# mueller-franzes/medfusion

Hardware: AMD Instinct MI355X
Metric: images/sec at 256x256, 150 DDIM steps (DiffusionPipeline.sample incl. VAE decode) (higher is better)
Workload: dtype f32 (emulated: fp16 pairs -- 23-bit operands, and 23-bit STORAGE of the tensors between the UNet's conv blocks: they exist as fp16 pairs only)

## Files before the change

### include/medfusion_hip.h

```cpp
#ifndef MEDFUSION_HIP_H
#define MEDFUSION_HIP_H

#include <stddef.h>
#include <stdint.h>

#ifdef __cplusplus
extern "C" {
#endif

#define MF_VERSION 250

enum { MF_OK = 0, MF_EINVAL = -1, MF_EUNSUPPORTED = -2, MF_ELAUNCH = -3, MF_EWORKSPACE = -4 };
enum { MF_LAYOUT_NHWC = 0, MF_LAYOUT_NCHW = 1 };

int mf_version(void);
const char* mf_last_error(void);

typedef struct MfConvDesc {
  int32_t N, Hin, Win;
  int32_t C1, C2;
  int32_t Cout;
  int32_t KH, KW;
  int32_t stride;
  int32_t pad;
  int32_t upsample;
  int32_t in_layout;
  int32_t out_layout;
  int32_t tile_hint;
  int32_t splitk_hint;
  int32_t precision;
} MfConvDesc;
enum { MF_CONV_FP32 = 0, MF_CONV_FP32_SPLIT3_W3 = 3, MF_CONV_BF16 = 4, MF_CONV_FP32_F16X2 = 5, MF_CONV_F16 = 6 };

int mf_pack_conv_weight_f32(const float* w_oihw, float* w_packed, int Cout, int Cin, int KH, int KW, void* stream);
int mf_pack_upconv_weight_f32(const float* w_oihw, float* w_packed, int Cout, int Cin, void* stream);
int mf_conv2d_subpixel_ok(const MfConvDesc* d);
int mf_conv2d_is_igemm(const MfConvDesc* d);
int mf_split_conv_weight_bf16x3(const float* w_packed, void* w_split, long rows, int K, void* stream);
int mf_convert_conv_weight_bf16(const float* w_packed, void* w_bf16, long rows, int K, void* stream);
size_t mf_conv2d_workspace_bytes(const MfConvDesc* d);
int mf_conv2d_f32(const float* x1, const float* x2, const float* w_packed, const float* bias, float* y,
                  void* workspace, size_t workspace_bytes, const MfConvDesc* d, void* stream);

int mf_conv2d_f16x2_ok(const MfConvDesc* d);
int mf_conv2d_f16x2_bound_slots(const MfConvDesc* d);
int mf_split_f16x2(const float* x, void* xs, const float* bound, int rows, int64_t per_row, void* stream);
int mf_split_f16x2_slots(const float* x, void* xs, const float* slots, int nslots, float* bound_out, int rows, int64_t per_row, void* stream);
int mf_conv2d_f16x2_sync_words(const MfConvDesc* d);
int mf_conv2d_f16x2(const void* x1s, const void* x2s, const void* ws, const float* bias, float* y, const float* x1_bound,
                    const float* x2_bound, float w_bound, float* y_bound, void* workspace, size_t workspace_bytes, uint32_t* sync,
                    double* gn_partial, int G, const MfConvDesc* d, void* stream);
int mf_conv2d_plan_query(const MfConvDesc* d, int32_t* tile_id, int32_t* splitk);
int mf_conv2d_plan_override(const MfConvDesc* d, int tile, int splitk);

typedef struct MfConvF16x2Call {
  const void* x1s; const void* x2s; const void* ws; const float* bias; float* y;
  const float* x1_bound; const float* x2_bound; float w_bound; float* y_bound;
  void* workspace; size_t workspace_bytes; uint32_t* sync;
  double* gn_partial; int G;
  const MfConvDesc* d;
} MfConvF16x2Call;
int mf_conv2d_f16x2_group_ok(const MfConvDesc* a, int Ga, const MfConvDesc* b, int Gb);
int mf_conv2d_f16x2_group(const MfConvF16x2Call* a, const MfConvF16x2Call* b, void* stream);

typedef struct MfGnFuse {
  const float* gamma;
  const float* beta;
  const float* residual;
  const void* residual_pairs;
  const float* res_bound;
  const float* res_bound_slots;
  const float* emb;
  const float* emb_bound;
  float* out;
  void* out_split;
  float* out_bound;
  uint32_t* rendezvous;
  uint32_t* error_flag;
  int64_t emb_stride;
  int32_t res_nslots;
  int32_t act;
  float bconst;
  float eps;
} MfGnFuse;
int mf_conv2d_f16x2_fuse_words(const MfConvDesc* d, int G);
int mf_conv2d_f16x2_gn_apply(const void* x1s, const void* x2s, const void* ws, const float* bias, const float* x1_bound, const float* x2_bound,
                             float w_bound, void* workspace, size_t workspace_bytes, uint32_t* sync, double* gn_partial, int G,
                             const MfGnFuse* f, const MfConvDesc* d, void* stream);

int mf_pack_nchw_pairs_f32(const float* x, void* out_pairs, float* bound_out, int N, int C, int HW, int CP, void* stream);
int mf_conv2d_f16x2_pairs_out_ok(const MfConvDesc* d);
int mf_conv2d_f16x2_pairs_out(const void* x1s, const void* x2s, const void* ws, const float* bias, float* y, void* y_split, float* y_bound_out,
                              const float* x1_bound, const float* x2_bound, float w_bound, float w_l1_1, float w_l1_2, float bias_max,
                              void* workspace, size_t workspace_bytes, uint32_t* sync, const MfConvDesc* d, void* stream);

int mf_wino_ok(const MfConvDesc* d);
int mf_wino_preferred(const MfConvDesc* d);
int mf_wino_in_table(const MfConvDesc* d);
int mf_wino_pack_weight_f32(const float* w_oihw, float* u, int Cout, int Cin, void* stream);
int mf_wino_input_f16x2(const void* xs, const float* x_bound, void* vs, float* v_bound, int N, int H, int W, int C, void* stream);
size_t mf_wino_workspace_bytes(const MfConvDesc* d);
int mf_wino_sync_words(const MfConvDesc* d);
int mf_wino_gn_parts(const MfConvDesc* d, int G);
int mf_wino_plan_query(const MfConvDesc* d, int32_t* tile_id, int32_t* splitk);
int mf_wino_f32_ok(const MfConvDesc* d, int G);
int mf_wino_input_f32(const float* x, float* v, int N, int H, int W, int C, void* stream);
int mf_wino_tail_f32(const float* m, const float* bias, const float* gamma, const float* beta, const float* residual, const float* emb, int64_t emb_stride,
                     float* out, float* out_wino, int N, int H, int W, int C, int G, int act, float eps, void* stream);
int mf_conv2d_wino_f16x2(const void* v1s, const void* v2s, const void* us, const float* bias, float* y, const float* v1_bound, const float* v2_bound,
                         float u_bound, void* workspace, size_t workspace_bytes, uint32_t* sync, double* gn_partial, int G, const MfConvDesc* d,
                         void* stream);
typedef struct MfWinoTail {
  const float* gamma; const float* beta;
  const float* residual; const void* residual_pairs;
  const float* res_bound; const float* res_bound_slots;
  const float* emb; const float* emb_bound;
  float* out; void* out_split; float* out_bound;
  void* out_wino; float* wino_bound;
  int64_t emb_stride;
  int32_t res_nslots, act;
  float bconst, eps;
} MfWinoTail;
int mf_wino_tail_ok(const MfConvDesc* d, int G);
int mf_wino_group_ok(const MfConvDesc* d, const MfConvDesc* guest);
int mf_conv2d_wino_gn_apply_f16x2(const void* v1s, const void* v2s, const void* us, const float* bias, const float* v1_bound, const float* v2_bound,
                                  float u_bound, void* workspace, size_t workspace_bytes, uint32_t* sync, int G, const MfWinoTail* t,
                                  const MfConvF16x2Call* guest, const MfConvDesc* d, void* stream);

int mf_conv2d_gn_parts(const MfConvDesc* d, int G);
int mf_conv2d_gn_f32(const float* x1, const float* x2, const float* w_packed, const float* bias, float* y, void* workspace,
                     size_t workspace_bytes, double* gn_partial, int G, const MfConvDesc* d, void* stream);

size_t mf_gn_stats_workspace_bytes(int N, int HW, int C, int G);
int mf_gn_stats_f32(const float* x, float* stats, void* workspace, size_t workspace_bytes, int N, int HW, int C, int G,
                    float eps, void* stream);
int mf_gn_partial_parts(int HW);
int mf_gn_stats_partial_f32(const float* x, double* partial, int N, int HW, int C, int G, void* stream);
int mf_gn_finalize_f32(const double* partial, int parts, float* stats, int N, int HW, int C, int G, float eps, void* stream);
int mf_gn_apply_f32(const float* x, const float* stats, const float* gamma, const float* beta, const float* residual,
                    const float* emb, int64_t emb_stride, float* out, int N, int HW, int C, int G, int act, void* stream);
int mf_gn_apply_split_f32(const float* x, const float* stats, const float* gamma, const float* beta, const float* residual,
                          const float* emb, int64_t emb_stride, float* out, void* out_split, const float* x_bound, const float* res_bound,
                          const float* emb_bound, float bconst, float* out_bound, int N, int HW, int C, int G, int act, void* stream);
int mf_gn_apply_from_partials_f32(const float* x, const double* gn_partial, int parts, float eps, const float* gamma, const float* beta,
                                  const float* residual, const float* emb, int64_t emb_stride, float* out, void* out_split,
                                  const float* res_bound, const float* res_bound_slots, int res_nslots, const float* emb_bound, float bconst,
                                  float* out_bound, int N, int HW, int C, int G, int act, void* stream);
int mf_gn_apply_from_partials_pairs_f32(const float* x, const double* gn_partial, int parts, float eps, const float* gamma, const float* beta,
                                        const float* residual, const void* residual_pairs, const float* emb, int64_t emb_stride, float* out,
                                        void* out_split, const float* res_bound, const float* res_bound_slots, int res_nslots,
                                        const float* emb_bound, float bconst, float* out_bound, int N, int HW, int C, int G, int act, void* stream);
int mf_maxabs_rows_slots(int64_t per_row);
int mf_maxabs_rows_f32(const float* x, float* partial, float* bound, int N, int64_t per_row, void* stream);
int mf_bound_finalize_f32(const float* partial, float* bound, int N, int slots, void* stream);

int mf_linear_f32(const float* x, int64_t x_stride, const float* w, const float* bias, float* y, int64_t y_stride,
                  int B, int In, int Out, int act_in, int act_out, int accumulate, void* stream);
int mf_sinusoidal_f32(const float* t, const float* freqs, float* out, int B, int dim, float max_period, float shift, int flip, void* stream);
int mf_learned_sinusoidal_f32(const float* t, const float* weights, float* out, int B, int emb_dim, void* stream);
int mf_embedding_add_f32(const float* table, const int64_t* idx, float* io, int B, int D, int num_rows, void* stream);

typedef struct MfSchedStep {
  float sqrt_recip_ac;
  float sqrt_recipm1_ac;
  float coef1, coef2;
  float std_fixed;
  float log_var_min;
  float log_var_max;
  float ddim_sqrt_an;
  float ddim_c;
  float ddim_sigma;
  int32_t t;
  int32_t mode;
} MfSchedStep;

typedef struct MfSchedArgs {
  const float* x_t;
  const float* pred;
  const float* pred_uncond;
  const float* pred_var;
  const float* noise_post;
  const float* noise_ddim;
  int64_t noise_step_stride;
  float* x_t_out;
  float* x0_out;
  float* xT_out;
  const MfSchedStep* table;
  const int32_t* step_dev;
  int32_t step;
  int32_t objective;
  int32_t clip_x0;
  float guidance_scale;
  int64_t n;
} MfSchedArgs;
int mf_sched_step_f32(const MfSchedArgs* a, void* stream);
int mf_sched_step_philox_f32(const MfSchedArgs* a, uint64_t seed, int32_t draw_base, int32_t draw_stride, int64_t sample_offset, int B,
                             int32_t* step_counter, uint32_t* ticket, void* stream);
typedef struct MfSchedBlend {
  const float* z0;
  const float* eps0;
  const uint8_t* mask;
  const float* coef;
  int64_t cells;
  int32_t channels;
  int32_t reserved;
} MfSchedBlend;
int mf_sched_step_blend_f32(const MfSchedArgs* a, const MfSchedBlend* blend, void* stream);
int mf_sched_step_philox_blend_f32(const MfSchedArgs* a, uint64_t seed, int32_t draw_base, int32_t draw_stride, int64_t sample_offset, int B,
                                   int32_t* step_counter, uint32_t* ticket, const MfSchedBlend* blend, void* stream);
enum { MF_SOLVER_FINAL = 0, MF_SOLVER_DDIM0 = 1, MF_SOLVER_ORDER1 = 2, MF_SOLVER_ORDER2 = 3 };
typedef struct MfSolverStep {
  float sqrt_recip_ac;
  float sqrt_recipm1_ac;
  float A, B, C;
  int32_t t;
  int32_t mode;
  int32_t reserved;
} MfSolverStep;
typedef struct MfSolverArgs {
  const float* x_t;
  const float* pred;
  const float* pred_uncond;
  float* x_t_out;
  float* x0_out;
  float* xT_out;
  float* x0_hist;
  const MfSolverStep* table;
  int32_t* step_counter;
  uint32_t* ticket;
  const int32_t* step_dev;
  int32_t step;
  int32_t objective;
  int32_t clip_x0;
  float guidance_scale;
  int64_t n;
} MfSolverArgs;
int mf_solver_step_f32(const MfSolverArgs* a, void* stream);
int mf_solver_step_blend_f32(const MfSolverArgs* a, const MfSchedBlend* blend, void* stream);
int mf_select_cells_f32(const uint8_t* mask, const float* a, const float* b, float* out, int N, int C, int64_t cells, void* stream);
int mf_mask_maxpool_u8(const void* mask, int mask_is_f32, uint8_t* out, int N, int D, int H, int W, int fd, int fh, int fw, void* stream);
int mf_broadcast_from_table_f32(const float* table, const int32_t* step_dev, int32_t step, float* out, int n, void* stream);
int mf_gather_step_rows_f32(const float* table, const int64_t* cols, const int32_t* step_dev, int32_t step, int ncol, int64_t row_len,
                            float* out, int B, void* stream);
int mf_gather_step_rows3_f32(const float* const* tables, const int64_t* row_lens, float* const* outs, int n_tables, const int64_t* cols,
                             const int32_t* step_dev, int32_t step, int ncol, int B, void* stream);
int mf_counter_add_i32(int32_t* counter, int32_t inc, void* stream);

int mf_rows_axpby_f32(const float* x, const float* y, const float* a, const float* c, const float* d, float* out, int B,
                      int64_t per_row, int do_clamp, float lo, float hi, void* stream);

int mf_philox_normal_f32(float* out, uint64_t seed, int32_t draw_base, int32_t draw_stride, const int32_t* step_dev,
                         int32_t step, int64_t sample_offset, int B, int64_t per_sample, void* stream);

int mf_attention_f32(const float* q, const float* k, const float* v, float* out, int B, int H, int Nq, int Nk, int d,
                     float scale, void* stream);
int mf_layernorm_f32(const float* x, const float* gamma, const float* beta, float* out, int64_t rows, int C, float eps,
                     void* stream);
int mf_geglu_f32(const float* h, float* out, int64_t rows, int C, void* stream);
int mf_add_f32(const float* a, const float* b, float* out, int64_t n, void* stream);

int mf_nchw_to_nhwc_f32(const float* x, float* y, int N, int C, int H, int W, void* stream);
int mf_nhwc_to_nchw_f32(const float* x, float* y, int N, int C, int H, int W, void* stream);
int mf_diag_gaussian_sample_f32(const float* moments, const float* noise, float* z, int N, int C, int HW, void* stream);
int mf_diag_gaussian_kl_f32(const float* moments, float* kl, int N, int C, int HW, void* stream);

size_t mf_vq_workspace_bytes(int64_t pixels);
int mf_vector_quantize_f32(const float* z, const float* codebook, float* z_q, int32_t* idx, double* sqerr, void* workspace,
                           size_t workspace_bytes, int N, int C, int HW, int K, void* stream);

typedef struct MfConv3dDesc {
  int32_t N, D, H, W;
  int32_t C1, C2;
  int32_t Cout;
  int32_t k;
  int32_t stride[3];
  int32_t pad[3];
  int32_t upsample[3];
  int32_t tile_hint;
  int32_t splitk_hint;
  int32_t precision;
// ... 40 lines not shown
```

### medfusion_amd/blocks.py

```python
from __future__ import annotations

import os
from typing import Optional, Tuple, Union

import torch
import torch.nn as nn

from . import kernels as K
from . import lib as L

Act = Union[torch.Tensor, Tuple[torch.Tensor, torch.Tensor]]


def monai_padding(kernel_size: int, stride: int) -> int:
    p = (kernel_size - stride + 1) / 2
    if p < 0:
        raise AssertionError("padding value should not be negative")
    return int(p)


def zero_module(m: nn.Module) -> nn.Module:
    for p in m.parameters():
        p.detach().zero_()
    return m


def _split(x: Act):
    return (x[0], x[1]) if isinstance(x, (tuple, list)) else (x, None)


class _Packed:

    def __init__(self, subpixel: bool = False, pad_cin: int = 0):
        self._pad_cin = pad_cin
        self._key = None
        self._w = None
        self._w3 = None
        self._wb = None
        self._wh = None
        self._wu = None
        self._l1 = {}
        self._subpixel = subpixel

    def get(self, weight: torch.Tensor) -> torch.Tensor:
        key = (weight.data_ptr(), weight._version, weight.device)
        if key != self._key:
            w = weight.detach()
            if w.dim() == 3:
                w = w.unsqueeze(-1)
            if self._pad_cin and w.shape[1] < self._pad_cin:
                w = torch.nn.functional.pad(w, (0, 0, 0, 0, 0, self._pad_cin - w.shape[1]))
            self._w = K.pack_upconv_weight(w) if self._subpixel else K.pack_conv_weight(w)
            self._w3 = None
            self._wb = None
            self._wh = None
            self._wu = None
            self._l1 = {}
            self._raw = w
            self._key = key
        return self._w

    def get_wino(self, weight: torch.Tensor):
        self.get(weight)
        if self._wu is None:
            self._wu = K.split_weight_f16x2(K.wino_pack_weight(self._raw))
        return self._wu

    def get_wino_f32(self, weight: torch.Tensor, split3: bool):
        self.get(weight)
        if getattr(self, "_wuf_key", None) != self._key:
            self._wuf, self._wu3, self._wuf_key = K.wino_pack_weight(self._raw), None, self._key
        if not split3:
            return self._wuf
        if self._wu3 is None:
            self._wu3 = K.split_conv_weight(self._wuf)
        return self._wu3

    def get_f16x2(self, weight: torch.Tensor) -> torch.Tensor:
        wp = self.get(weight)
        if self._wh is None:
            self._wh = K.split_weight_f16x2(wp)
        return self._wh

    def l1(self, weight: torch.Tensor, c1: int):
        wp = self.get(weight)
        ent = self._l1.get(c1)
        if ent is None:
            a = wp[..., :c1].abs().sum(dim=(-3, -2, -1)).max()
            b = wp[..., c1:].abs().sum(dim=(-3, -2, -1)).max() if c1 < wp.shape[-1] else torch.zeros((), device=wp.device)
            ent = self._l1[c1] = (float(a.item()) * (1.0 + 1e-5), float(b.item()) * (1.0 + 1e-5))
        return ent

    def get_bf16(self, weight: torch.Tensor) -> torch.Tensor:
        wp = self.get(weight)
        if self._wb is None:
            self._wb = K.convert_conv_weight_bf16(wp)
        return self._wb

    def get_split(self, weight: torch.Tensor) -> torch.Tensor:
        wp = self.get(weight)
        if self._w3 is None:
            self._w3 = K.split_conv_weight(wp)
        return self._w3


PAIRS_ONLY_BETWEEN_BLOCKS = os.environ.get("MEDFUSION_PAIRS_ONLY", "1") != "0"
INPUT_CONV_ON_PAIRS = os.environ.get("MEDFUSION_INPUT_CONV_PAIRS", "0") == "1"
GROUPED_CONV_RES = os.environ.get("MEDFUSION_GROUPED_CONV_RES", "1") != "0"
GROUP_GUEST = {}
DERIVED_OUT_BOUNDS = os.environ.get("MEDFUSION_DERIVED_BOUNDS", "1") != "0"
SUBPIXEL_UPSAMPLE = True
CONV_PRECISION = int(os.environ.get("MEDFUSION_CONV_PRECISION", "5"))
WINOGRAD = int(os.environ.get("MEDFUSION_WINOGRAD", "1"))


WINOGRAD_F32 = int(os.environ.get("MEDFUSION_WINOGRAD_F32", "1"))
WINOGRAD_F32_MFMA = int(os.environ.get("MEDFUSION_WINOGRAD_F32_MFMA", "0"))
WINO_TAIL = os.environ.get("MEDFUSION_WINOGRAD_TAIL", "1") != "0"
WINO_GROUP = os.environ.get("MEDFUSION_WINOGRAD_GROUP", "1") != "0"
WINO_SHAPES = {}
if os.environ.get("MEDFUSION_WINOGRAD_TABLE"):
    import json as _json
    WINO_SHAPES = {tuple(e[:5]): (int(e[5]), int(e[6])) for e in _json.load(open(os.environ["MEDFUSION_WINOGRAD_TABLE"]))}


def wino_wanted(d) -> bool:
    if WINOGRAD == 0:
        return False
    if (d.N, d.Hin, d.Win, d.C1 + d.C2, d.Cout) in WINO_SHAPES:
        return K.wino_ok(d)
    return K.wino_ok(d) if WINOGRAD == 2 else K.wino_preferred(d)


def f16x2_mode() -> bool:
    return CONV_PRECISION in (5, 6)


class Conv(nn.Module):

    def __init__(self, in_ch, out_ch, kernel_size, stride=1, padding=0, upsample=False, conv1d=False):
        super().__init__()
        holder = nn.Conv1d(in_ch, out_ch, 1) if conv1d else nn.Conv2d(in_ch, out_ch, kernel_size, stride, padding, bias=True)
        self.weight, self.bias = holder.weight, holder.bias
        self.in_ch, self.out_ch, self.k, self.stride, self.pad, self.upsample = in_ch, out_ch, kernel_size, stride, padding, int(upsample)
        self._packed = _Packed()
        self._packed_sub = _Packed(subpixel=True)
        self._packed_pad = _Packed(pad_cin=32)
        self._pad_ok = {}
        self._descs = {}
        self._pairs_out = {}
        self._wino_sites = {}
        self._bmax = (None, 0.0)

    def _forward_f16x2(self, x1, x2, n, h, w, c1, c2, out, gn_groups, gn_eps, measure_out, prec=5, derive_out=False, cin_pad=0):
        key = ("f16x2", n, h, w, c1, c2, gn_groups, prec, WINOGRAD)
        ent = self._descs.get(key)
        if ent is None:
            d = K.make_conv_desc(n, h, w, c1, c2, self.out_ch, self.k, self.stride, self.pad, 2 if self.upsample else 0, precision=prec)
            ok = K.conv_f16x2_ok(d)
            pinned = K.pin_conv_plan(d) if ok else None
            wino = None
            if ok and prec == 5 and not cin_pad and self.k == 3 and wino_wanted(d):
                wparts = K.wino_gn_parts(d, gn_groups) if gn_groups else 0
                if not gn_groups or wparts > 0:
                    wt, wsk = WINO_SHAPES.get((n, h, w, c1 + c2, self.out_ch), (0, 0))
                    wd = K.make_conv_desc(n, h, w, c1, c2, self.out_ch, self.k, self.stride, self.pad, 0, tile_hint=wt, splitk_hint=wsk, precision=prec)
                    wino = (wd, wparts, K.pin_wino_plan(wd))
            ent = (d, K.conv_gn_parts(d, gn_groups) if (ok and gn_groups) else 0, ok, pinned, wino)
            self._descs[key] = ent
        d, parts, ok, pinned, wino = ent
        if not ok:
            return None
        if wino is not None and out is None and not measure_out and not derive_out:
            wd, wparts, wpinned = wino
            r = K.conv2d_wino_f16x2(x1, self._packed.get_wino(self.weight), self.bias, wd, x2=x2, gn_groups=gn_groups, gn_parts=wparts, pinned=wpinned)
            return (r[0], K.GnPartials(r[1], wparts, gn_eps)) if gn_groups else r
        pk = self._packed_pad if cin_pad else (self._packed_sub if d.upsample == 2 else self._packed)
        wh = pk.get_f16x2(self.weight)
        if not gn_groups:
            if derive_out and out is None and DERIVED_OUT_BOUNDS:
                po = self._pairs_out.get(key)
                if po is None:
                    po = self._pairs_out[key] = K.conv_pairs_out_ok(d)
                if po:
                    bkey = (self.bias._version, self.bias.data_ptr())
                    if self._bmax[0] != bkey:
                        self._bmax = (bkey, float(self.bias.detach().abs().max().item()))
                    return K.conv2d_f16x2_pairs_out(x1, wh, self.bias, d, pk.l1(self.weight, c1), self._bmax[1], x2=x2, pinned=pinned)
            return K.conv2d_f16x2(x1, wh, self.bias, d, x2=x2, out=out, measure_out=measure_out, pinned=pinned)
        ho, wo = K.conv_out_hw(d)
        if parts > 0:
            y, partial = K.conv2d_f16x2(x1, wh, self.bias, d, x2=x2, out=out, gn_groups=gn_groups, gn_parts=parts, pinned=pinned)
        else:
            y = K.conv2d_f16x2(x1, wh, self.bias, d, x2=x2, out=out, pinned=pinned)
            partial, parts = K.gn_stats_partial(y, gn_groups)
        if gn_groups <= 256:
            return y, K.GnPartials(partial, parts, gn_eps)
        return y, K.gn_finalize(partial, parts, ho * wo, self.out_ch, gn_groups, gn_eps)

    def wino_tail_desc(self, x: Act, G: int):
        x1, x2 = _split(x)
        n, h, w, c1 = x1.shape
        c2 = 0 if x2 is None else x2.shape[-1]
        key = ("wino_tail", n, h, w, c1, c2, G, WINOGRAD, WINO_TAIL)
        ent = self._descs.get(key)
        if ent is None:
            ent = False
            if WINO_TAIL and CONV_PRECISION == 5 and self.k == 3 and self.stride == 1 and not self.upsample and c1 + c2 == self.in_ch:
                d = K.make_conv_desc(n, h, w, c1, c2, self.out_ch, self.k, self.stride, self.pad, 0, precision=5)
                if wino_wanted(d) and K.wino_tail_ok(d, G):
                    wt, wsk = WINO_SHAPES.get((n, h, w, c1 + c2, self.out_ch), (0, 0))
                    d.tile_hint, d.splitk_hint = wt, wsk
                    ent = (d, K.pin_wino_plan(d))
            self._descs[key] = ent
        return (key, ent) if ent is not False else (key, None)

    def forward_wino_gn_apply(self, x: Act, norm, act: int, residual, emb, emb_stride, out_fp32, bconst, guest=None):
        x1, x2 = _split(x)
        n, h, w, c1 = x1.shape
        c2 = 0 if x2 is None else x2.shape[-1]
        if c1 + c2 != self.in_ch:
            raise RuntimeError(f"conv expects {self.in_ch} input channels, got {c1}+{c2}")
        G = norm.num_groups
        key, ent = self.wino_tail_desc(x, G)
        if ent is None:
            return None
        d, pinned = ent
        want = self._wino_sites.get(key, False)
        y = K.conv2d_wino_gn_apply(x1, self._packed.get_wino(self.weight), self.bias, d, norm.weight, norm.bias, G, norm.eps, act=act, residual=residual,
                                   emb=emb, emb_stride=emb_stride, x2=x2, bconst=bconst, out_fp32=out_fp32, want_wino=want, pinned=pinned, guest=guest)
        if not want:
            y._mf_wino_site = (self._wino_sites, key)
        return y

    def forward_wino_gn_apply_f32(self, x: Act, norm, act: int, residual, emb, emb_stride, split3: bool = True):
        x1, x2 = _split(x)
        n, h, w, c1 = x1.shape
        c2 = 0 if x2 is None else x2.shape[-1]
        G = norm.num_groups
        mode = WINOGRAD_F32 if split3 else WINOGRAD_F32_MFMA
        key = ("wino_f32", n, h, w, c1, c2, G, mode, split3)
        ent = self._descs.get(key)
        if ent is None:
            ent = False
            if self.k == 3 and self.stride == 1 and not self.upsample and c1 + c2 == self.in_ch:
                d = K.make_conv_desc(n, h, w, c1, c2, self.out_ch, 3, 1, 1, 0, precision=3 if split3 else 0)
                if K.wino_f32_ok(d, G) and K.conv_is_igemm(d):
                    rule = K.make_conv_desc(n, h, w, c1, c2, self.out_ch, 3, 1, 1, 0, precision=5)
                    if mode == 2 or h * w <= 256 or K.wino_preferred(rule):
                        ent = d
            self._descs[key] = ent
        if ent is False:
            return None
        K._need_f32(x1, x2, residual)
        want = self._wino_sites.get(key, False)
        y = K.conv2d_wino_gn_apply_f32(x1, self._packed.get_wino_f32(self.weight, split3), self.bias, ent, norm.weight, norm.bias, G, norm.eps, act=act,
                                       residual=residual, emb=emb, emb_stride=emb_stride, x2=x2, want_wino=want)
        if not want:
            y._mf_wino_site_f32 = (self._wino_sites, key)
        return y

    def forward_gn_apply(self, x: Act, norm, act: int, residual, emb, emb_stride, out_fp32, bconst):
        x1, x2 = _split(x)
        n, h, w, c1 = x1.shape
        c2 = 0 if x2 is None else x2.shape[-1]
        if c1 + c2 != self.in_ch:
            raise RuntimeError(f"conv expects {self.in_ch} input channels, got {c1}+{c2}")
        prec = CONV_PRECISION
        G = norm.num_groups
        key = ("fused", n, h, w, c1, c2, G, prec)
        ent = self._descs.get(key)
        if ent is None:
# ... 547 lines not shown
```

### medfusion_amd/csrc/conv_f16x2.h

```cpp
#pragma once
#include "common.h"
#include "split_f16.h"

#ifndef MFC2_HZ
#define MFC2_HZ 0
#endif
#ifndef MFC2_OUT_STORE
#define MFC2_OUT_STORE 0
#endif

namespace mfc2 {
using namespace mf;

typedef float f32x16 __attribute__((ext_vector_type(16)));
typedef float f32x4 __attribute__((ext_vector_type(4)));
typedef unsigned int u32x4 __attribute__((ext_vector_type(4)));
typedef _Float16 f16x8 __attribute__((ext_vector_type(8)));
typedef _Float16 f16x2 __attribute__((ext_vector_type(2)));

struct FuseP {
  int on, act;
  float eps, bconst;
  double count;
  const float* gamma;
  const float* beta;
  const float* res_f32;
  const void* res_pairs;
  const float* res_bound;
  const float* res_slots;
  int res_nslots;
  int tiles_per_sample;
  const float* emb;
  long emb_stride;
  const float* emb_bound;
  float* out_f32;
  void* out_pairs;
  float* out_bound;
  unsigned* rv;
  unsigned* rv_err;
};

struct ConvP2 {
  const void* x1;
  const void* x2;
  const void* w;
  const float* bias;
  float* y;
  const float* bound1;
  const float* bound2;
  int wexp;
  float* out_bound;
  int bound_slots;
  int N, Hin, Win, C1, C2, Cin, Cout;
  int Hout, Wout, Heff, Weff, KH, KW, stride, pad;
  int M, K, HWout;
  int cgroups, cg_per_split, splitk;
  int tiles_m, tiles_n;
  long slab;
  unsigned bytes1, bytes2, bytesw;
  int subpix, hw_src;
  int out_nt;
  int wphase_rows;
  int walk_n_fast;
  double* gn_partial;
  int gn_groups, gn_parts, gn_cpg;
  int tree;
  float* handoff;
  unsigned* sync;
  FuseP fz;
  void* y_pairs;
  float* y_pair_bound;
  float wl1_1, wl1_2, bmax;
#if MFC2_HZ & (256 | 512)
  float* dbg;
#endif
};

__device__ __forceinline__ int xcd_remap2(int bid, int total) {
  const int q = total >> 3, r = total & 7;
  const int xcd = bid & 7, within = bid >> 3;
  const int base = xcd < r ? xcd * (q + 1) : r * (q + 1) + (xcd - r) * q;
  return base + within;
}

#ifndef MFC2_HZ
#define MFC2_HZ 0
#endif
#define MFC2_HZ_ON(BIT) ((MFC2_HZ >> (BIT)) & 1)
#ifndef MFC2_HZ_PAD
#define MFC2_HZ_PAD 7
#endif

__device__ __forceinline__ float hz_add(float a, float b) { float r; asm volatile("v_add_f32 %0, %1, %2" : "=v"(r) : "v"(a), "v"(b)); return r; }
__device__ __forceinline__ float hz_mul(float a, float b) { float r; asm volatile("v_mul_f32 %0, %1, %2" : "=v"(r) : "v"(a), "v"(b)); return r; }

#define MFC2_WAIT_VM(N) asm volatile("s_waitcnt vmcnt(%0)" ::"n"(N) : "memory")
#if MFC2_HZ & 512
#define MFC2_STAMP(I) { if (p.dbg && threadIdx.x == 0) reinterpret_cast<unsigned long*>(p.dbg)[(long)MFC2_BID * 8 + (I)] = __builtin_amdgcn_s_memrealtime(); }
#else
#define MFC2_STAMP(I)
#endif
#define MFC2_WAIT_LGKM0() asm volatile("s_waitcnt lgkmcnt(0)" ::: "memory")

#define MFC2_BODY_AS_KERNEL 1
#define MFC2_BID blockIdx.x
#include "conv_f16x2_body.inc"
#undef MFC2_BODY_AS_KERNEL
#undef MFC2_BID
#define MFC2_BODY_AS_KERNEL 0
#define MFC2_BID bid
#include "conv_f16x2_body.inc"
#undef MFC2_BODY_AS_KERNEL
#undef MFC2_BID

__global__ __launch_bounds__(256) void split_act_f16x2_kernel(const float* __restrict__ x, u32x4* __restrict__ out, long octets,
                                                              const float* __restrict__ bound, long octets_per_row) {
  const long stride = (long)gridDim.x * blockDim.x;
  for (long o = (long)blockIdx.x * blockDim.x + threadIdx.x; o < octets; o += stride) {
    const float sc = bound ? exp2i(-scale_exp_of(bound[o / octets_per_row])) : 1.f;
    const f32x4 v0 = *reinterpret_cast<const f32x4*>(x + o * 8) * sc, v1 = *reinterpret_cast<const f32x4*>(x + o * 8 + 4) * sc;
    u32x4 hi, lo;
    split8_f16(v0, v1, hi, lo);
    out[o * 2] = hi;
    out[o * 2 + 1] = lo;
  }
}

__global__ __launch_bounds__(256) void split_act_slots_kernel(const float* __restrict__ x, u32x4* __restrict__ out, long octets_per_row,
                                                              const float* __restrict__ slots, int nslots, float* __restrict__ bound_out) {
  __shared__ float sm[4];
  const int row = blockIdx.y, tid = threadIdx.x;
  float m = 0.f;
  for (int i = tid; i < nslots; i += 256) m = fmaxf(m, slots[(long)row * nslots + i]);
  m = mf::wave_max(m);
  if ((tid & 63) == 0) sm[tid >> 6] = m;
  __syncthreads();
  const float b = fmaxf(fmaxf(sm[0], sm[1]), fmaxf(sm[2], sm[3]));
  if (blockIdx.x == 0 && tid == 0) bound_out[row] = b;
  const float sc = exp2i(-scale_exp_of(b));
  const long base = (long)row * octets_per_row;
  for (long o = (long)blockIdx.x * 256 + tid; o < octets_per_row; o += (long)gridDim.x * 256) {
    const f32x4 v0 = *reinterpret_cast<const f32x4*>(x + (base + o) * 8) * sc, v1 = *reinterpret_cast<const f32x4*>(x + (base + o) * 8 + 4) * sc;
    u32x4 hi, lo;
    split8_f16(v0, v1, hi, lo);
    out[(base + o) * 2] = hi;
    out[(base + o) * 2 + 1] = lo;
  }
}

}
```

### medfusion_amd/csrc/conv_f16x2.hip

```cpp
#include "common.h"
#include <string.h>
#include <mutex>
#include <vector>
#include "gn_partial.h"
#include "conv_plan.h"
#include "conv_f16x2.h"
#include "conv_f16x2_halo.h"
#include "conv_f16x2_group.h"
#include "winograd.h"

using namespace mf;

namespace {

struct Tile2 { int id, BM, BN, WM, WN, NST, HG; };
const Tile2 kTiles2[] = {
    {31, 128, 256, 2, 4, 3, 0}, {32, 256, 128, 4, 2, 3, 0}, {33, 128, 128, 2, 4, 3, 0}, {34, 128, 128, 4, 2, 3, 0}, {35, 256, 64, 4, 2, 3, 0},
    {36, 128, 64, 4, 2, 3, 0}, {37, 64, 256, 1, 8, 3, 0},
    {51, 128, 128, 2, 2, 2, 0}, {52, 128, 128, 2, 2, 3, 0}, {53, 64, 128, 2, 2, 3, 0}, {54, 128, 64, 2, 2, 3, 0},
    {61, 256, 128, 4, 2, 3, 6}, {62, 256, 128, 4, 2, 3, 7}, {63, 128, 128, 2, 4, 3, 4}, {64, 128, 128, 2, 4, 3, 5},
};
inline size_t tile_lds(const Tile2& t) {
  return t.HG ? (size_t)2 * t.HG * (t.WM * t.WN) * 1024 + (size_t)3 * t.BN * 128 : (size_t)t.NST * (t.BM + t.BN) * 128;
}
// ... 305 lines not shown
}

static int bound_slots2(const MfConvDesc* d, const Plan2& pl, bool with_stats) {
  const int HW = pl.Hout * pl.Wout;
  if (pl.splitk == 1 || tree_possible(d, pl)) {
    if (!tile_sample_aligned(pl)) return 0;
    const int nw = pl.t.WM * pl.t.WN;
    return HW >= pl.t.BM ? (HW / pl.t.BM) * (d->Cout / pl.t.BN) * nw : (d->Cout / pl.t.BN) * (nw * HW / pl.t.BM);
  }
  if (with_stats) return 0;
  const long p4 = (long)HW * d->Cout / 4;
  int bx = (int)((p4 + 255) / 256);
  const int cap = cdiv(2048, d->N);
  if (bx > cap) bx = cap;
  return bx * 4;
}

int mf_conv2d_f16x2_bound_slots(const MfConvDesc* d) {
  Plan2 pl;
  if (!d || !pair_precision(d->precision) || make_plan2(d, &pl) != MF_OK || !pl.ok) return 0;
  return bound_slots2(d, pl, false);
}

int mf_conv2d_plan_query(const MfConvDesc* d, int32_t* tile_id, int32_t* splitk) {
  MF_REQUIRE(d, MF_EINVAL, "plan_query: null desc");
  if (pair_precision(d->precision)) {
    Plan2 pl;
    int rc = make_plan2(d, &pl);
    if (rc) return rc;
    if (tile_id) *tile_id = pl.ok ? pl.t.id : 0;
    if (splitk) *splitk = pl.ok ? pl.splitk : 0;
    return MF_OK;
  }
  return igemm_plan_query(d, tile_id, splitk);
}

int mf_split_f16x2(const float* x, void* xs, const float* bound, int rows, int64_t per_row, void* stream) {
  MF_REQUIRE(x && xs && rows > 0 && per_row > 0 && per_row % 8 == 0, MF_EINVAL, "split_f16x2: bad args (per_row %% 8 == 0)");
  const long octets = (long)rows * (per_row / 8);
  ProfScope ps(MF_FAM_MISC, (hipStream_t)stream, 0, 8.0 * rows * (double)per_row);
  const int blocks = (int)((octets + 255) / 256 > 8192 ? 8192 : (octets + 255) / 256);
  MF_LAUNCH(mfc2::split_act_f16x2_kernel, dim3(blocks), dim3(256), 0, (hipStream_t)stream, x, reinterpret_cast<mfc2::u32x4*>(xs), octets, bound,
                     (long)(per_row / 8));
  return check_launch("split_f16x2");
}

int mf_split_f16x2_slots(const float* x, void* xs, const float* slots, int nslots, float* bound_out, int rows, int64_t per_row, void* stream) {
  MF_REQUIRE(x && xs && slots && bound_out && nslots > 0 && rows > 0 && rows <= 65535 && per_row > 0 && per_row % 8 == 0, MF_EINVAL,
             "split_f16x2_slots: bad args (per_row %% 8 == 0, rows <= 65535)");
  const long opr = per_row / 8;
  ProfScope ps(MF_FAM_MISC, (hipStream_t)stream, 0, 8.0 * rows * (double)per_row);
  long bpr = (opr + 255) / 256;
  const long cap = (8192 + rows - 1) / rows;
  if (bpr > cap) bpr = cap;
  MF_LAUNCH(mfc2::split_act_slots_kernel, dim3((int)bpr, rows), dim3(256), 0, (hipStream_t)stream, x, reinterpret_cast<mfc2::u32x4*>(xs), opr, slots, nslots,
            bound_out);
  return check_launch("split_f16x2_slots");
}

static int host_scale_exp(float bound) {
  if (!(bound > 0.f)) return 0;
  uint32_t u;
  memcpy(&u, &bound, 4);
  const int s = (int)((u >> 23) & 0xffu) - 127 - 14;
  return s < -100 ? -100 : (s > 100 ? 100 : s);
}

int mf_conv2d_plan_override(const MfConvDesc* d, int tile, int splitk) {
  MF_REQUIRE(d && pair_precision(d->precision), MF_EINVAL, "plan_override: a MF_CONV_FP32_F16X2 / MF_CONV_F16 descriptor");
  std::lock_guard<std::mutex> lk(g_plan_mu);
  const int Cin = d->C1 + d->C2;
  for (size_t i = 0; i < g_plan_overrides.size(); ++i) {
    const PlanEntry& e = g_plan_overrides[i];
    if (e.N == d->N && e.H == d->Hin && e.W == d->Win && e.Cin == Cin && e.Cout == d->Cout && e.k == d->KH && e.stride == d->stride && e.ups == d->upsample) {
      g_plan_overrides.erase(g_plan_overrides.begin() + i);
      break;
    }
  }
  if (tile > 0 && splitk > 0) g_plan_overrides.push_back(PlanEntry{d->N, d->Hin, d->Win, Cin, d->Cout, d->KH, d->stride, d->upsample, tile, splitk});
  return MF_OK;
}

int mf_conv2d_f16x2_sync_words(const MfConvDesc* d) {
  Plan2 pl;
  if (!d || !pair_precision(d->precision) || make_plan2(d, &pl) != MF_OK || !pl.ok || !tree_possible(d, pl)) return 0;
  return cdiv(pl.M, pl.t.BM) * (d->Cout / pl.t.BN) * (pl.splitk - 1);
}

static int fuse_tiles_per_sample(const MfConvDesc* d, const Plan2& pl, int G) {
  if (!pl.ok || G <= 0 || G > 256 || d->Cout % G || d->upsample != 0) return 0;
  if (pl.splitk > 1 && !tree_possible(d, pl)) return 0;
  if (!epilogue_stats_ok(d, pl, G)) return 0;
  const int HW = pl.Hout * pl.Wout;
  if (HW < pl.t.BM && pl.t.BM / HW > 8) return 0;
  const long grid = (long)cdiv(pl.M, pl.t.BM) * (d->Cout / pl.t.BN) * pl.splitk;
  mfc2::ConvP2 dummy{};
  const int resident = dispatch_tile(pl.t.id, dummy, nullptr, d->precision == MF_CONV_F16 ? 1 : 3, 1);
  if (resident <= 0 || grid > resident) return 0;
  static const int fault = [] { const char* e = getenv("MEDFUSION_FUSE_FAULT"); return e ? atoi(e) : 0; }();
  return (HW >= pl.t.BM ? HW / pl.t.BM : 1) * (d->Cout / pl.t.BN) + (fault ? 1 : 0);
}

int mf_conv2d_f16x2_fuse_words(const MfConvDesc* d, int G) {
  Plan2 pl;
  if (!d || !pair_precision(d->precision) || make_plan2(d, &pl) != MF_OK || !pl.ok) return 0;
  return fuse_tiles_per_sample(d, pl, G) > 0 ? 2 * d->N : 0;
}

struct PairsOut { void* y_split; float* y_bound; float wl1_1, wl1_2, bmax; };
static int conv_f16x2_impl(const void* x1s, const void* x2s, const void* ws, const float* bias, float* y, const float* x1_bound, const float* x2_bound,
                           float w_bound, float* y_bound, void* workspace, size_t workspace_bytes, uint32_t* sync, double* gn_partial, int G,
                           const MfGnFuse* fz, const MfConvDesc* d, void* stream, const PairsOut* po = nullptr);

int mf_conv2d_f16x2_pairs_out_ok(const MfConvDesc* d) {
  Plan2 pl;
  if (!d || !pair_precision(d->precision) || make_plan2(d, &pl) != MF_OK || !pl.ok || d->Cout % 8) return 0;
  return (pl.splitk == 1 || tree_possible(d, pl)) ? 1 : 0;
}

int mf_conv2d_f16x2_pairs_out(const void* x1s, const void* x2s, const void* ws, const float* bias, float* y, void* y_split, float* y_bound_out,
                              const float* x1_bound, const float* x2_bound, float w_bound, float w_l1_1, float w_l1_2, float bias_max, void* workspace,
                              size_t workspace_bytes, uint32_t* sync, const MfConvDesc* d, void* stream) {
  MF_REQUIRE(y && y_split && y_bound_out && x1_bound, MF_EINVAL, "conv(f16x2, pairs out): y, y_split, y_bound_out and x1_bound are required");
  MF_REQUIRE(d && (d->C2 == 0 || x2_bound), MF_EINVAL, "conv(f16x2, pairs out): x2_bound with a second source");
  MF_REQUIRE(mf_conv2d_f16x2_pairs_out_ok(d), MF_EUNSUPPORTED, "conv(f16x2, pairs out): this plan reduces split-K behind the launch (mf_conv2d_f16x2_pairs_out_ok == 0)");
  MF_REQUIRE(w_l1_1 >= 0.f && w_l1_2 >= 0.f && bias_max >= 0.f, MF_EINVAL, "conv(f16x2, pairs out): norms must be >= 0");
  const PairsOut po{y_split, y_bound_out, w_l1_1, w_l1_2, bias_max};
  return conv_f16x2_impl(x1s, x2s, ws, bias, y, x1_bound, x2_bound, w_bound, nullptr, workspace, workspace_bytes, sync, nullptr, 0, nullptr, d, stream, &po);
}

int mf_conv2d_f16x2(const void* x1s, const void* x2s, const void* ws, const float* bias, float* y, const float* x1_bound, const float* x2_bound,
                    float w_bound, float* y_bound, void* workspace, size_t workspace_bytes, uint32_t* sync, double* gn_partial, int G,
                    const MfConvDesc* d, void* stream) {
  MF_REQUIRE(y, MF_EINVAL, "conv(f16x2): null pointer");
  return conv_f16x2_impl(x1s, x2s, ws, bias, y, x1_bound, x2_bound, w_bound, y_bound, workspace, workspace_bytes, sync, gn_partial, G, nullptr, d, stream);
}

int mf_conv2d_f16x2_gn_apply(const void* x1s, const void* x2s, const void* ws, const float* bias, const float* x1_bound, const float* x2_bound,
                             float w_bound, void* workspace, size_t workspace_bytes, uint32_t* sync, double* gn_partial, int G, const MfGnFuse* f,
                             const MfConvDesc* d, void* stream) {
  MF_REQUIRE(f && gn_partial && G > 0, MF_EINVAL, "conv_gn_apply: needs the fuse arguments, the record array and G");
  MF_REQUIRE(f->out_split && f->out_bound && f->rendezvous && f->error_flag, MF_EINVAL, "conv_gn_apply: out_split, out_bound, rendezvous and error_flag are required");
  MF_REQUIRE((f->gamma == nullptr) == (f->beta == nullptr), MF_EINVAL, "conv_gn_apply: gamma/beta must both be given or both NULL");
  MF_REQUIRE(!(f->residual && f->residual_pairs), MF_EINVAL, "conv_gn_apply: the residual is fp32 OR fp16 pairs");
  MF_REQUIRE(!f->residual_pairs || f->res_bound, MF_EINVAL, "conv_gn_apply: a residual given as fp16 pairs needs the res_bound that scaled it");
  MF_REQUIRE(!f->residual || f->res_bound || (f->res_bound_slots && f->res_nslots > 0), MF_EINVAL, "conv_gn_apply: a residual needs res_bound or res_bound_slots");
  MF_REQUIRE(!f->emb || (f->emb_bound && f->emb_stride % 4 == 0), MF_EINVAL, "conv_gn_apply: an embedding needs emb_bound and emb_stride %% 4 == 0");
  return conv_f16x2_impl(x1s, x2s, ws, bias, nullptr, x1_bound, x2_bound, w_bound, nullptr, workspace, workspace_bytes, sync, gn_partial, G, f, d, stream);
}

struct Prep { mfc2::ConvP2 p; Plan2 pl; bool tree; double flops, bytes; int terms; };
static int conv_f16x2_prepare(const void* x1s, const void* x2s, const void* ws, const float* bias, float* y, const float* x1_bound, const float* x2_bound,
                              float w_bound, float* y_bound, void* workspace, size_t workspace_bytes, uint32_t* sync, double* gn_partial, int G,
                              const MfGnFuse* fz, const MfConvDesc* d, const PairsOut* po, Prep* out, bool wino_gemm = false) {
  MF_REQUIRE(d && pair_precision(d->precision), MF_EINVAL, "conv(f16x2): desc.precision must be MF_CONV_FP32_F16X2 (or the opt-in MF_CONV_F16)");
  MF_REQUIRE((d->upsample == 3) == wino_gemm, MF_EINVAL, "conv(f16x2): upsample = 3 is internal to mf_conv2d_wino_f16x2");
  Plan2& pl = out->pl;
  mfc2::ConvP2& p = out->p;
  int rc = make_plan2(d, &pl);
  if (rc) return rc;
  MF_REQUIRE(pl.ok, MF_EUNSUPPORTED, "conv(f16x2): this shape/layout is not on the fp16-pair path (ask mf_conv2d_f16x2_ok)");
  MF_REQUIRE(x1s && ws && (y || fz), MF_EINVAL, "conv(f16x2): null pointer");
  MF_REQUIRE(d->C2 == 0 || x2s != nullptr, MF_EINVAL, "conv(f16x2): C2 > 0 but x2 is null");
  MF_REQUIRE(!gn_partial || gn_parts2(d, pl, G) > 0, MF_EUNSUPPORTED, "conv(f16x2): cannot emit GroupNorm partials (mf_conv2d_gn_parts == 0)");
  MF_REQUIRE(!y_bound || (!gn_partial && bound_slots2(d, pl, false) > 0), MF_EUNSUPPORTED,
             "conv(f16x2): cannot measure the output bound of this plan (mf_conv2d_f16x2_bound_slots == 0, or GroupNorm statistics requested)");
  p.x1 = x1s; p.x2 = x2s; p.w = ws; p.bias = bias; p.y = y;
  p.bound1 = x1_bound; p.bound2 = x2_bound; p.wexp = host_scale_exp(w_bound); p.out_bound = y_bound; p.bound_slots = y_bound ? bound_slots2(d, pl, false) : 0;
  p.N = d->N; p.Hin = d->Hin; p.Win = d->Win; p.C1 = d->C1; p.C2 = d->C2; p.Cin = d->C1 + d->C2; p.Cout = d->Cout;
  p.Hout = pl.Hout; p.Wout = pl.Wout; p.Heff = pl.Heff; p.Weff = pl.Weff;
  p.KH = d->KH; p.KW = d->KW; p.stride = d->stride; p.pad = d->pad;
  p.subpix = d->upsample == 2 ? 1 : 0; p.hw_src = d->Hin * d->Win;
  if (p.subpix) { p.KH = p.KW = 2; p.Heff = d->Hin; p.Weff = d->Win; }
  p.M = pl.M; p.K = pl.K; p.HWout = pl.Hout * pl.Wout;
  p.cgroups = pl.cgroups; p.cg_per_split = pl.cg_per_split; p.splitk = pl.splitk;
  p.tiles_m = cdiv(pl.M, pl.t.BM); p.tiles_n = d->Cout / pl.t.BN;
  p.slab = (long)pl.M * d->Cout;
  p.bytes1 = (unsigned)(4.0 * d->N * d->Hin * d->Win * d->C1);
  p.bytes2 = (unsigned)(4.0 * d->N * d->Hin * d->Win * d->C2);
  p.bytesw = (unsigned)(4.0 * d->Cout * pl.K * (p.subpix ? 4 : wino_gemm ? 16 : 1));
  p.wphase_rows = wino_gemm ? (d->N / 16) * d->Hin * d->Win : 0;
  {
    static const int walk = [] { const char* e = getenv("MF_CONV_WALK"); return e ? atoi(e) : 1; }();
    const double act_bytes = 4.0 * d->N * d->Hin * d->Win * (d->C1 + d->C2), w_bytes = 4.0 * d->Cout * pl.K * (p.subpix ? 4 : 1);
    p.walk_n_fast = (!wino_gemm && p.tiles_n > 1 && (walk == 2 || (walk == 1 && act_bytes > w_bytes))) ? 1 : 0;
  }
  p.out_nt = 0;
  p.gn_partial = nullptr; p.gn_groups = G; p.gn_cpg = G > 0 ? d->Cout / G : 8; p.gn_parts = 0;
  p.tree = 0; p.handoff = nullptr; p.sync = nullptr;
#if MFC2_HZ & (256 | 512)
  p.dbg = g_conv_dbg;
#endif
  p.y_pairs = po ? po->y_split : nullptr; p.y_pair_bound = po ? po->y_bound : nullptr;
  p.wl1_1 = po ? po->wl1_1 : 0.f; p.wl1_2 = po ? po->wl1_2 : 0.f; p.bmax = po ? po->bmax : 0.f;
  memset(&p.fz, 0, sizeof(p.fz));
  if (fz) {
    const int tps = fuse_tiles_per_sample(d, pl, G);
    MF_REQUIRE(tps > 0, MF_EUNSUPPORTED, "conv_gn_apply: this plan cannot apply its GroupNorm inside the launch (mf_conv2d_f16x2_fuse_words == 0)");
    p.fz.on = 1; p.fz.act = fz->act; p.fz.eps = fz->eps; p.fz.bconst = fz->bconst; p.fz.count = (double)(pl.Hout * pl.Wout) * (d->Cout / G);
    p.fz.gamma = fz->gamma; p.fz.beta = fz->beta; p.fz.res_f32 = fz->residual; p.fz.res_pairs = fz->residual_pairs;
    p.fz.res_bound = fz->res_bound; p.fz.res_slots = fz->res_bound ? nullptr : fz->res_bound_slots; p.fz.res_nslots = fz->res_nslots;
    p.fz.tiles_per_sample = tps; p.fz.emb = fz->emb; p.fz.emb_stride = (long)fz->emb_stride; p.fz.emb_bound = fz->emb_bound;
    p.fz.out_f32 = fz->out; p.fz.out_pairs = fz->out_split; p.fz.out_bound = fz->out_bound; p.fz.rv = fz->rendezvous; p.fz.rv_err = fz->error_flag;
  }
  const bool tree = pl.splitk > 1 && tree_possible(d, pl) && (!gn_partial || epilogue_stats_ok(d, pl, G));
  if ((pl.splitk == 1 || tree) && gn_partial) { p.gn_partial = gn_partial; p.gn_parts = p.HWout >= pl.t.BM ? p.HWout / pl.t.BM : 1; }
  if (tree) {
    const size_t need = tree_handoff_bytes(d, pl);
    MF_REQUIRE(workspace && workspace_bytes >= need, MF_EWORKSPACE, "conv(f16x2): workspace %zu < %zu", workspace_bytes, need);
    MF_REQUIRE(sync, MF_EINVAL, "conv(f16x2): this plan meets its split-K slices inside the launch and needs `sync` "
                                "(mf_conv2d_f16x2_sync_words(d) zero-initialised words the caller keeps between launches)");
    p.tree = tree_mode(); p.handoff = reinterpret_cast<float*>(workspace); p.sync = sync;
    if (y_bound && p.bound_slots == 0) p.out_bound = nullptr;
  } else if (pl.splitk > 1) {
    const size_t need = (size_t)pl.splitk * pl.M * d->Cout * sizeof(float);
    MF_REQUIRE(workspace && workspace_bytes >= need, MF_EWORKSPACE, "conv(f16x2): workspace %zu < %zu", workspace_bytes, need);
    p.y = reinterpret_cast<float*>(workspace);
    p.out_bound = nullptr;
  }
  out->tree = tree;
  out->flops = 2.0 * pl.M * (double)d->Cout * (d->upsample == 2 ? 9.0 * (d->C1 + d->C2) : (double)pl.K);
  out->bytes = 4.0 * ((double)d->N * d->Hin * d->Win * p.Cin + (double)d->Cout * pl.K + (double)pl.M * d->Cout);
  out->terms = d->precision == MF_CONV_F16 ? 1 : 3;
  return MF_OK;
}

static int conv_f16x2_impl(const void* x1s, const void* x2s, const void* ws, const float* bias, float* y, const float* x1_bound, const float* x2_bound,
                           float w_bound, float* y_bound, void* workspace, size_t workspace_bytes, uint32_t* sync, double* gn_partial, int G,
                           const MfGnFuse* fz, const MfConvDesc* d, void* stream, const PairsOut* po) {
  Prep q;
  int rc = conv_f16x2_prepare(x1s, x2s, ws, bias, y, x1_bound, x2_bound, w_bound, y_bound, workspace, workspace_bytes, sync, gn_partial, G, fz, d, po, &q);
  if (rc) return rc;
  hipStream_t s = (hipStream_t)stream;
  const Plan2& pl = q.pl;
  const mfc2::ConvP2& p = q.p;
  const bool tree = q.tree;
  {
    const int terms = q.terms;
    ProfScope ps(fz ? MF_FAM_CONV_GN_FUSED : MF_FAM_CONV_IGEMM, s, q.flops, q.bytes, 2.0 * pl.M * (double)d->Cout * pl.K * terms);
    ps.set_tag(pl.t.id + (terms == 1 ? 100000 : 0));
    rc = dispatch_tile(pl.t.id, p, s, terms, 0);
    if (rc == -1) { set_error("conv(f16x2): no tile config %d", pl.t.id); rc = MF_EINVAL; }
  }
  if (rc) return rc;
  if (pl.splitk > 1 && !tree) {
    const int HW = p.HWout;
    ProfScope ps(MF_FAM_SPLITK_REDUCE, s, 0, 4.0 * pl.M * d->Cout * (pl.splitk + 1));
    if (gn_partial) {
      const int slices = stats_slices(d->N, HW, d->Cout, G), chunks = stats_chunks(HW);
      MF_LAUNCH(gn_partial_kernel<true>, dim3(chunks, d->N, slices), dim3(kStatsThreads), stats_lds_bytes(d->Cout / slices), s,
                         reinterpret_cast<const float*>(workspace), gn_partial, HW, d->Cout, G, pl.splitk, p.slab, bias, y, (float*)nullptr);
      return check_launch("splitk_reduce_stats");
    }
    const long p4 = (long)HW * d->Cout / 4;
    int bx = (int)((p4 + 255) / 256);
    const int cap = cdiv(2048, d->N);
    if (bx > cap) bx = cap;
    MF_LAUNCH(splitk_reduce_kernel<0>, dim3(bx, d->N), dim3(256), 0, s, reinterpret_cast<const float*>(workspace), bias, y, p4, d->Cout,
                       pl.splitk, p.slab, y_bound);
    return check_launch("splitk_reduce");
  }
  return MF_OK;
}

static bool single_launch(const MfConvDesc* d, const Plan2& pl, int G) {
  if (pl.splitk == 1) return G == 0 || gn_parts2(d, pl, G) > 0;
  return tree_possible(d, pl) && (G == 0 || epilogue_stats_ok(d, pl, G));
}

int mf_conv2d_f16x2_group_ok(const MfConvDesc* a, int Ga, const MfConvDesc* b, int Gb) {
  static const int off = [] { const char* e = getenv("MF_CONV_GROUP"); return e && atoi(e) == 0 ? 1 : 0; }();
  if (off || !a || !b || a->precision != MF_CONV_FP32_F16X2 || b->precision != MF_CONV_FP32_F16X2) return 0;
  Plan2 pa, pb;
  if (make_plan2(a, &pa) != MF_OK || make_plan2(b, &pb) != MF_OK || !pa.ok || !pb.ok) return 0;
  if (!single_launch(a, pa, Ga) || !single_launch(b, pb, Gb)) return 0;
  mfc2::ConvP2 dummy{};
  return dispatch_group(pa.t.id, pb.t.id, dummy, dummy, nullptr, 2) == 1 ? 1 : 0;
}

int mf_conv2d_f16x2_group(const MfConvF16x2Call* a, const MfConvF16x2Call* b, void* stream) {
  MF_REQUIRE(a && b && a->d && b->d && a->y && b->y, MF_EINVAL, "conv_group: two calls with descriptors and outputs");
  const int Ga = a->gn_partial ? a->G : 0, Gb = b->gn_partial ? b->G : 0;
  MF_REQUIRE(mf_conv2d_f16x2_group_ok(a->d, Ga, b->d, Gb), MF_EUNSUPPORTED,
             "conv_group: these two plans cannot share a launch (mf_conv2d_f16x2_group_ok == 0: a reducer pass behind one of them, workgroup sizes "
             "that differ, or a tile pair that is not instantiated)");
  Prep qa, qb;
  int rc = conv_f16x2_prepare(a->x1s, a->x2s, a->ws, a->bias, a->y, a->x1_bound, a->x2_bound, a->w_bound, a->y_bound, a->workspace, a->workspace_bytes,
                              a->sync, a->gn_partial, a->G, nullptr, a->d, nullptr, &qa);
  if (rc) return rc;
  rc = conv_f16x2_prepare(b->x1s, b->x2s, b->ws, b->bias, b->y, b->x1_bound, b->x2_bound, b->w_bound, b->y_bound, b->workspace, b->workspace_bytes,
                          b->sync, b->gn_partial, b->G, nullptr, b->d, nullptr, &qb);
  if (rc) return rc;
  MF_REQUIRE((qa.pl.splitk == 1 || qa.tree) && (qb.pl.splitk == 1 || qb.tree), MF_EUNSUPPORTED, "conv_group: a plan needs its reducer pass");
  if (qa.tree && qb.tree) {
    const char *wa = (const char*)a->workspace, *wb = (const char*)b->workspace;
    const size_t na = tree_handoff_bytes(a->d, qa.pl), nb = tree_handoff_bytes(b->d, qb.pl);
    MF_REQUIRE(wa + na <= wb || wb + nb <= wa, MF_EINVAL, "conv_group: the two workspaces overlap");
    const uint32_t *sa = a->sync, *sb = b->sync;
    const long ca = mf_conv2d_f16x2_sync_words(a->d), cb = mf_conv2d_f16x2_sync_words(b->d);
    MF_REQUIRE(sa + ca <= sb || sb + cb <= sa, MF_EINVAL, "conv_group: the two sync arrays overlap");
  }
  MF_REQUIRE(a->y != b->y, MF_EINVAL, "conv_group: one output for two convolutions");
  hipStream_t s = (hipStream_t)stream;
  ProfScope ps(MF_FAM_CONV_IGEMM, s, qa.flops + qb.flops, qa.bytes + qb.bytes,
               2.0 * 3.0 * (qa.pl.M * (double)a->d->Cout * qa.pl.K + qb.pl.M * (double)b->d->Cout * qb.pl.K));
  ps.set_tag(1000 + 100 * qa.pl.t.id + qb.pl.t.id);
  rc = dispatch_group(qa.pl.t.id, qb.pl.t.id, qa.p, qb.p, s, 0);
  if (rc == -1) { set_error("conv_group: no tile pair (%d, %d)", qa.pl.t.id, qb.pl.t.id); rc = MF_EINVAL; }
  return rc;
}

int mf_prof_tag_name(int family, int tag, char* buf, int n) {
  MF_REQUIRE(buf && n > 0, MF_EINVAL, "mf_prof_tag_name: bad args");
  auto tile_of = [](int id) -> const Tile2* { for (const auto& k : kTiles2) if (k.id == id) return &k; return nullptr; };
  auto tile_type = [&](int id, char* o, int m) {
    const Tile2* t = tile_of(id);
    if (!t) { snprintf(o, m, "?"); return; }
    if (t->HG) snprintf(o, m, "mfc2::HaloTile<%d, %d, %d, %d, %d>", t->BM, t->BN, t->WM, t->WN, t->HG);
    else snprintf(o, m, "mfc2::PlainTile<%d, %d, %d, %d, %d>", t->BM, t->BN, t->WM, t->WN, t->NST);
  };
  if ((family == MF_FAM_CONV_IGEMM || family == MF_FAM_CONV_GN_FUSED) && tag > 0) {
    const int terms = tag >= 100000 ? 1 : 3, id = tag % 100000;
    if (id >= 1000) {
      char a[96], b[96];
      tile_type((id - 1000) / 100, a, sizeof a);
      tile_type((id - 1000) % 100, b, sizeof b);
      snprintf(buf, n, "void mfc2::conv_group_kernel<%s, %s, 3>(mfc2::ConvP2, mfc2::ConvP2, int)", a, b);
      return MF_OK;
    }
    if (const Tile2* t = tile_of(id)) {
      if (t->HG) snprintf(buf, n, "void mfc2::conv_halo_kernel<%d, %d, %d, %d, %d, %d>(mfc2::ConvP2)", t->BM, t->BN, t->WM, t->WN, t->HG, terms);
      else snprintf(buf, n, "void mfc2::conv_f16x2_kernel<%d, %d, %d, %d, %d, %d>(mfc2::ConvP2)", t->BM, t->BN, t->WM, t->WN, t->NST, terms);
      return MF_OK;
    }
// ... 9 lines not shown
```

### medfusion_amd/csrc/conv_f16x2_body.inc

```
template <int BM, int BN, int WM, int WN, int NST, int TERMS = 3>
#if MFC2_BODY_AS_KERNEL
__global__ __launch_bounds__(WM * WN * 64, 2) void conv_f16x2_kernel(const ConvP2 p) {
#else
__device__ __forceinline__ void conv_f16x2_body(const ConvP2& p, const int bid) {
#endif
  static_assert(TERMS == 3 || TERMS == 1, "three product terms (fp16 pairs) or one (fp16)");
  constexpr int PC = TERMS == 3 ? 2 : 1;
  constexpr int NW = WM * WN;
  static_assert(NW == 8 || NW == 4, "4 or 8 waves");
  constexpr int FM = BM / WM, FN = BN / WN, TM = FM / 32, TN = FN / 32;
  static_assert(TM >= 1 && TN >= 1 && FM % 32 == 0 && FN % 32 == 0, "per-wave footprint");
  constexpr int GP = BM / (8 * NW), GQ = BN / (8 * NW), NL = GP + GQ;
  static_assert(BM % (8 * NW) == 0 && BN % (8 * NW) == 0, "tile");
  constexpr int ROWB = 128, STAGE = (BM + BN) * ROWB;
  constexpr int NM = TERMS * TM * TN;
  constexpr int NR = PC * (TM + TN);
  constexpr int NF = (2 * NM + 2) / 3;
  static_assert(NST >= 2 && NST <= 6 && NST * STAGE <= 160 * 1024 && (NST - 1) * NL <= 63, "LDS stages");
  static_assert((NR + NF - 1) / NF <= 3, "at most three reads per slot");

  extern __shared__ __attribute__((aligned(1024))) char smem[];
  MFC2_STAMP(0)

  const int tid = threadIdx.x, lane = tid & 63;
  const int wave = __builtin_amdgcn_readfirstlane(tid >> 6);
  const int wm = wave / WN, wn = wave % WN;

  const int total = p.tiles_m * p.tiles_n * p.splitk;
  const int logical = xcd_remap2(MFC2_BID, total);
  int tile_m = logical % p.tiles_m;
  const int rest = logical / p.tiles_m;
  int tile_n = rest % p.tiles_n;
  int kz = rest / p.tiles_n;
  if (p.walk_n_fast) {
    tile_n = logical % p.tiles_n;
    const int r1 = logical / p.tiles_n;
    tile_m = r1 % p.tiles_m;
    kz = r1 / p.tiles_m;
  }
  if (p.wphase_rows) {
    const int tpc = p.wphase_rows / BM, ncomp = p.tiles_m / tpc;
    const int tm_in = logical % tpc, r1 = logical / tpc;
    tile_n = r1 % p.tiles_n;
    const int r2 = r1 / p.tiles_n;
    tile_m = (r2 % ncomp) * tpc + tm_in;
    kz = r2 / ncomp;
  }
  const int m0 = tile_m * BM, n0 = tile_n * BN;
  const int cg_beg = kz * p.cg_per_split;
  const int cg_end = min(p.cgroups, cg_beg + p.cg_per_split);
  const int taps = p.KH * p.KW;
  const int nit = (cg_end - cg_beg) * taps;

  const int lrow = lane >> 3;
  const unsigned slot16 = (unsigned)(((lane & 7) ^ ((4 * (wave & 1) + (lane >> 4)) & 7)) * 16);
  int a_pix[GP], a_inv[GP];
  const bool small_m = p.M < (1 << 23);
  const float r_hw = 1.0f / (float)p.HWout, r_w = 1.0f / (float)(p.subpix ? p.Win : p.Wout), r_src = 1.0f / (float)p.hw_src;
  auto qdiv = [small_m](int a, int d, float rd) {
    if (!small_m) return a / d;
    int q = (int)((float)a * rd);
    const int r = a - q * d;
    q += (r >= d ? 1 : 0) - (r < 0 ? 1 : 0);
    return q;
  };
#pragma unroll
  for (int i = 0; i < GP; ++i) {
    const int m = m0 + 8 * (wave + NW * i) + lrow;
    int n_ = 0, iy0 = -(1 << 28), ix0 = 0;
    if (m < p.M) {
      const int n = qdiv(m, p.HWout, r_hw);
      const int rem = m - n * p.HWout;
      n_ = n * p.Hin;
      if (p.subpix) {
        const int ph = qdiv(rem, p.hw_src, r_src), r2 = rem - ph * p.hw_src;
        const int y = qdiv(r2, p.Win, r_w), x = r2 - y * p.Win;
        iy0 = y + (ph >> 1) - 1;
        ix0 = x + (ph & 1) - 1;
      } else {
        const int oy = qdiv(rem, p.Wout, r_w), ox = rem - oy * p.Wout;
        iy0 = oy * p.stride - p.pad;
        ix0 = ox * p.stride - p.pad;
      }
    }
    unsigned vy = 0, vx = 0;
#pragma unroll
    for (int t = 0; t < 3; ++t) {
      vy |= (t < p.KH && (unsigned)(iy0 + t) < (unsigned)p.Heff ? 1u : 0u) << t;
      vx |= (t < p.KW && (unsigned)(ix0 + t) < (unsigned)p.Weff ? 1u : 0u) << t;
    }
    const unsigned valid = ((vy & 1u) ? vx : 0u) | ((vy & 2u) ? vx << p.KW : 0u) | ((vy & 4u) ? vx << (2 * p.KW) : 0u);
    a_inv[i] = (int)~valid;
    a_pix[i] = (n_ + iy0) * p.Win + ix0;
  }
  const __amdgpu_buffer_rsrc_t rsw = __builtin_amdgcn_make_buffer_rsrc(const_cast<void*>(p.w), 0, p.bytesw, 0x00020000);
  const int phase_t = p.subpix ? ((m0 % p.HWout) / p.hw_src) : (p.wphase_rows ? m0 / p.wphase_rows : 0);
  const unsigned kbytes = (unsigned)p.K * 4u;
  const unsigned qv = (unsigned)(phase_t * p.Cout + n0 + 8 * wave + lrow) * kbytes + slot16;

  int l_cc = cg_beg, l_ky = 0, l_kx = 0, l_it = 0, l_st = 0;
  unsigned pbase[GP], l_off[GP];
  unsigned l_cs4 = 0, l_so = 0;
  int l_lds = 0;
  __amdgpu_buffer_rsrc_t l_rs = rsw;

#define MFC2_CHUNK_SETUP()                                                                                              \
  {                                                                                                                     \
    const int c0_ = l_cc * 32;                                                                                          \
    const bool first_ = c0_ < p.C1;                                                                                     \
    l_cs4 = (unsigned)(first_ ? p.C1 : p.C2) * 4u;                                                                      \
    const unsigned cb4_ = (unsigned)(first_ ? c0_ : c0_ - p.C1) * 4u + slot16;                                          \
    l_rs = __builtin_amdgcn_make_buffer_rsrc(const_cast<void*>(first_ ? p.x1 : p.x2), 0, first_ ? p.bytes1 : p.bytes2, 0x00020000); \
    _Pragma("unroll") for (int i = 0; i < GP; ++i) pbase[i] = (unsigned)a_pix[i] * l_cs4 + cb4_;                        \
  }
#define MFC2_LOAD_PREP()                                                                                                \
  {                                                                                                                     \
    const unsigned ts_ = (unsigned)(l_ky * p.KW + l_kx);                                                                \
    const unsigned tapb_ = (unsigned)(l_ky * p.Win + l_kx) * l_cs4;                                                     \
    _Pragma("unroll") for (int i = 0; i < GP; ++i) l_off[i] = (pbase[i] + tapb_) | (unsigned)__builtin_amdgcn_sbfe(a_inv[i], ts_, 1u); \
    l_so = (ts_ * (unsigned)p.Cin + (unsigned)l_cc * 32u) * 4u;                                                         \
    l_lds = l_st * STAGE + wave * 1024;                                                                                 \
  }
#define MFC2_LOAD_UNIT(U)                                                                                               \
  {                                                                                                                     \
    constexpr int u_ = (U);                                                                                             \
    if constexpr (u_ < GP) {                                                                                            \
      const unsigned off_ = l_off[u_];    \
      __builtin_amdgcn_raw_ptr_buffer_load_lds(l_rs, (__attribute__((address_space(3))) void*)(smem + l_lds + NW * u_ * 1024), 16, off_, 0, 0, 0); \
    } else {                                                                                                            \
      constexpr int q_ = u_ - GP;                                                                                       \
      __builtin_amdgcn_raw_ptr_buffer_load_lds(rsw, (__attribute__((address_space(3))) void*)(smem + l_lds + BM * ROWB + NW * q_ * 1024), 16, qv, \
                                               l_so + (unsigned)q_ * (8u * NW) * kbytes, 0, 0);                         \
    }                                                                                                                   \
  }
#define MFC2_LOAD_ADVANCE()                  \
  {                                          \
    ++l_it;                                  \
    l_st = l_st == NST - 1 ? 0 : l_st + 1;   \
    ++l_kx;                                  \
    if (l_kx == p.KW) { l_kx = 0; ++l_ky; }  \
    if (l_ky == p.KH) {                      \
      l_ky = 0;                              \
      ++l_cc;                                \
      if (l_it < nit) MFC2_CHUNK_SETUP()     \
    }                                        \
  }
#define MFC2_LOAD_ALL()                                            \
  {                                                                \
    MFC2_LOAD_PREP()                                               \
    MFC2_LOAD_UNIT(0) MFC2_LOAD_UNIT(1)                            \
    if constexpr (NL > 2) MFC2_LOAD_UNIT(NL > 2 ? 2 : 0)           \
    if constexpr (NL > 3) MFC2_LOAD_UNIT(NL > 3 ? 3 : 0)           \
    if constexpr (NL > 4) MFC2_LOAD_UNIT(NL > 4 ? 4 : 0)           \
    if constexpr (NL > 5) MFC2_LOAD_UNIT(NL > 5 ? 5 : 0)           \
    if constexpr (NL > 6) MFC2_LOAD_UNIT(NL > 6 ? 6 : 0)           \
    if constexpr (NL > 7) MFC2_LOAD_UNIT(NL > 7 ? 7 : 0)           \
  }

  const int fkey = (lane >> 1) & 7, fh = lane >> 5;
  int foff[2][2];
#pragma unroll
  for (int s = 0; s < 2; ++s)
#pragma unroll
    for (int c = 0; c < 2; ++c) foff[s][c] = (lane & 31) * ROWB + (((4 * s + 2 * fh + c) ^ fkey) * 16);
  const int xrow0 = wm * FM * ROWB;
  const int wrow0 = BM * ROWB + wn * FN * ROWB;

  f32x16 accm[TM][TN], accx[TM][TN];
#pragma unroll
  for (int i = 0; i < TM; ++i)
#pragma unroll
    for (int j = 0; j < TN; ++j)
#pragma unroll
      for (int r = 0; r < 16; ++r) { accm[i][j][r] = 0.f; accx[i][j][r] = 0.f; }

  f16x8 fx[2][TM][2], fw[2][TN][2];

  const bool first_src1 = cg_beg * 32 < p.C1, last_src2 = (cg_end - 1) * 32 >= p.C1;
  const int it_sw = __builtin_amdgcn_readfirstlane((first_src1 && last_src2) ? (p.C1 / 32 - cg_beg) * taps : -1);
#ifndef MFC2_EXPS_EARLY
#define MFC2_EXPS_EARLY 1
#endif
#if MFC2_EXPS_EARLY
#define MFC2_PIXEL_EXPS_DECL()                                                                                          \
  float pb1[TM] = {}, pb2[TM] = {};    \
  f32x4 eb0 = {0.f, 0.f, 0.f, 0.f}, eb1 = {0.f, 0.f, 0.f, 0.f};
#define MFC2_PIXEL_EXPS_LOAD()                                                                                          \
  _Pragma("unroll") for (int i = 0; i < TM; ++i) {                                                                      \
    const int pm_ = min(m0 + wm * FM + i * 32 + (lane & 31), p.M - 1);                                                  \
    const int pn_ = pm_ / p.HWout;                                                                                      \
    pb1[i] = p.bound1 ? p.bound1[pn_] : 0.f;                                                                            \
    pb2[i] = (p.bound2 && p.C2 > 0) ? p.bound2[pn_] : 0.f;                                                              \
  }                                                                                                                     \
  if ((p.splitk == 1 || p.tree) && p.bias) {                                                                            \
    const int bc0_ = n0 + wn * FN + (lane % (FN / 8)) * 8;                                                              \
    eb0 = *reinterpret_cast<const f32x4*>(p.bias + bc0_);                                                               \
    eb1 = *reinterpret_cast<const f32x4*>(p.bias + bc0_ + 4);                                                           \
  }
#define MFC2_PIXEL_EXPS(I) const int e1_ = p.bound1 ? scale_exp_of(pb1[I]) : 0, e2_ = (p.bound2 && p.C2 > 0) ? scale_exp_of(pb2[I]) : 0;
#else
#define MFC2_PIXEL_EXPS_DECL()
#define MFC2_PIXEL_EXPS_LOAD()
#define MFC2_PIXEL_EXPS(I)                                                                                              \
    const int pm_ = min(m0 + wm * FM + (I) * 32 + (lane & 31), p.M - 1);                                                \
    const int pn_ = pm_ / p.HWout;                                                                                      \
    const int e1_ = p.bound1 ? scale_exp_of(p.bound1[pn_]) : 0;                                                         \
    const int e2_ = (p.bound2 && p.C2 > 0) ? scale_exp_of(p.bound2[pn_]) : 0;
#endif
  MFC2_PIXEL_EXPS_DECL()
#define MFC2_SOURCE_SWITCH()                                                                                            \
  if (__builtin_expect(it == it_sw, 0)) {                                                                               \
    if constexpr (MFC2_HZ_ON(0)) asm volatile("s_nop 15\n\ts_nop 15" ::: "memory");                                     \
    _Pragma("unroll") for (int i = 0; i < TM; ++i) {                                                                    \
      MFC2_PIXEL_EXPS(i)                                                                                                \
      const float f_ = exp2i(e1_) * exp2i(-e2_);                                                                        \
      _Pragma("unroll") for (int j = 0; j < TN; ++j)                                                                    \
        _Pragma("unroll") for (int r = 0; r < 16; ++r) { accm[i][j][r] *= f_; accx[i][j][r] *= f_; }                    \
    }                                                                                                                   \
  }

#define MFC2_READ_UNIT(S, SB, U)                                                                                        \
  {                                                                                                                     \
    constexpr int u_ = (U);                                                                                             \
    if constexpr (u_ < PC * TM) {                                                                                       \
      fx[S][u_ / PC][u_ % PC] = *reinterpret_cast<const f16x8*>(smem + (SB) + xrow0 + (u_ / PC) * 32 * ROWB + foff[S][u_ % PC]); \
    } else {                                                                                                            \
      constexpr int v_ = u_ - PC * TM;                                                                                  \
      fw[S][v_ / PC][v_ % PC] = *reinterpret_cast<const f16x8*>(smem + (SB) + wrow0 + (v_ / PC) * 32 * ROWB + foff[S][v_ % PC]); \
    }                                                                                                                   \
  }
#define MFC2_MFMA(S, N_)                                                                                                \
  {                                                                                                                     \
    constexpr int n_ = (N_);                                                                                            \
    constexpr int j_ = n_ % TN, i_ = (n_ / TN) % TM, t_ = n_ / (TN * TM);                                               \
    if constexpr (t_ == 0) accm[i_][j_] = __builtin_amdgcn_mfma_f32_32x32x16_f16(fw[S][j_][0], fx[S][i_][0], accm[i_][j_], 0, 0, 0); \
    if constexpr (t_ == 1) accx[i_][j_] = __builtin_amdgcn_mfma_f32_32x32x16_f16(fw[S][j_][0], fx[S][i_][PC - 1], accx[i_][j_], 0, 0, 0); \
    if constexpr (t_ == 2) accx[i_][j_] = __builtin_amdgcn_mfma_f32_32x32x16_f16(fw[S][j_][PC - 1], fx[S][i_][0], accx[i_][j_], 0, 0, 0); \
  }

  if (nit > 0) {
    MFC2_CHUNK_SETUP()
    MFC2_LOAD_ALL()
    MFC2_LOAD_ADVANCE()
#pragma unroll
    for (int k = 1; k < NST; ++k)
      if (nit > k) { MFC2_LOAD_ALL() MFC2_LOAD_ADVANCE() }
    MFC2_PIXEL_EXPS_LOAD()
    {
      const int g = min(nit, NST) - 1;
      if (g >= 5) { MFC2_WAIT_VM(5 * NL <= 63 ? 5 * NL : 0); } else if (g == 4) { MFC2_WAIT_VM(4 * NL <= 63 ? 4 * NL : 0); }
      else if (g == 3) { MFC2_WAIT_VM(3 * NL); } else if (g == 2) { MFC2_WAIT_VM(2 * NL); } else if (g == 1) { MFC2_WAIT_VM(NL); } else { MFC2_WAIT_VM(0); }
    }
    __builtin_amdgcn_s_barrier();
    MFC2_STAMP(1)
    MFC2_READ_UNIT(0, 0, 0) MFC2_READ_UNIT(0, 0, 1)
    if constexpr (NR > 2) MFC2_READ_UNIT(0, 0, NR > 2 ? 2 : 0)
    if constexpr (NR > 3) MFC2_READ_UNIT(0, 0, NR > 3 ? 3 : 0)
    if constexpr (NR > 4) { MFC2_READ_UNIT(0, 0, NR > 4 ? 4 : 0) MFC2_READ_UNIT(0, 0, NR > 4 ? 5 : 0) }
    if constexpr (NR > 6) { MFC2_READ_UNIT(0, 0, NR > 6 ? 6 : 0) MFC2_READ_UNIT(0, 0, NR > 6 ? 7 : 0) }
  }

#define MFC2_SLOT_A(N_, SB)                                                                                             \
  {                                                                                                                     \
    MFC2_MFMA(0, N_)                                                                                                    \
    __builtin_amdgcn_sched_barrier(0);     \
    constexpr int lo_ = (N_) < NF ? ((N_) * NR + NF - 1) / NF : NR, hi_ = (N_) < NF ? (((N_) + 1) * NR + NF - 1) / NF : NR; \
    if constexpr (lo_ < hi_ && lo_ < NR) MFC2_READ_UNIT(1, SB, lo_ < NR ? lo_ : 0)                                      \
    if constexpr (lo_ + 1 < hi_ && lo_ + 1 < NR) MFC2_READ_UNIT(1, SB, lo_ + 1 < NR ? lo_ + 1 : 0)                      \
    if constexpr (lo_ + 2 < hi_ && lo_ + 2 < NR) MFC2_READ_UNIT(1, SB, lo_ + 2 < NR ? lo_ + 2 : 0)                      \
    if constexpr ((N_) == NM - 1) MFC2_LOAD_PREP()                    \
    __builtin_amdgcn_sched_barrier(0);                                                                                  \
  }
#define MFC2_SLOT_B(N_, SB, DO_LOAD)                                                                                    \
  {                                                                                                                     \
    MFC2_MFMA(1, N_)                                                                                                    \
    __builtin_amdgcn_sched_barrier(0);                                                                                  \
    constexpr int lo_ = (N_) < NF ? ((N_) * NR + NF - 1) / NF : NR, hi_ = (N_) < NF ? (((N_) + 1) * NR + NF - 1) / NF : NR; \
    if constexpr (lo_ < hi_ && lo_ < NR) MFC2_READ_UNIT(0, SB, lo_ < NR ? lo_ : 0)                                      \
    if constexpr (lo_ + 1 < hi_ && lo_ + 1 < NR) MFC2_READ_UNIT(0, SB, lo_ + 1 < NR ? lo_ + 1 : 0)                      \
    if constexpr (lo_ + 2 < hi_ && lo_ + 2 < NR) MFC2_READ_UNIT(0, SB, lo_ + 2 < NR ? lo_ + 2 : 0)                      \
    constexpr int ll_ = ((N_) * NL + NM - 1) / NM, lh_ = (((N_) + 1) * NL + NM - 1) / NM;                               \
    if (DO_LOAD) {                                                                                                      \
      if constexpr (ll_ < lh_ && ll_ < NL) MFC2_LOAD_UNIT(ll_ < NL ? ll_ : 0)                                           \
      if constexpr (ll_ + 1 < lh_ && ll_ + 1 < NL) MFC2_LOAD_UNIT(ll_ + 1 < NL ? ll_ + 1 : 0)                           \
      if constexpr (ll_ + 2 < lh_ && ll_ + 2 < NL) MFC2_LOAD_UNIT(ll_ + 2 < NL ? ll_ + 2 : 0)                           \
// ... 55 lines not shown
```

### medfusion_amd/csrc/conv_f16x2_wino.inc

```

static void wino_gemm_desc(const MfConvDesc* d, MfConvDesc* g) {
  *g = *d;
  g->N = 16 * d->N;
  g->Hin = 1;
  g->Win = (d->Hin / 2) * (d->Win / 2);
  g->KH = g->KW = 1;
  g->stride = 1;
  g->pad = 0;
  g->upsample = 3;
}
static bool wino_shape_ok(const MfConvDesc* d) {
  return d && d->precision == MF_CONV_FP32_F16X2 && d->KH == 3 && d->KW == 3 && d->stride == 1 && d->pad == 1 && d->upsample == 0 &&
         d->in_layout == MF_LAYOUT_NHWC && d->out_layout == MF_LAYOUT_NHWC && d->N > 0 && d->Hin >= 2 && d->Win >= 2 && d->Hin % 2 == 0 && d->Win % 2 == 0 &&
         d->C1 > 0 && d->C1 % 32 == 0 && d->C2 >= 0 && d->C2 % 32 == 0 && d->Cout % 64 == 0 && d->Cout <= 1024 && 256 % (d->Cout / 4) == 0 &&
         (double)d->N * 16.0 * (d->Hin / 2) * (d->Win / 2) < 2147483647.0;
}
static size_t wino_m_bytes(const MfConvDesc* d) {
  const size_t b = (size_t)16 * d->N * (d->Hin / 2) * (d->Win / 2) * d->Cout * sizeof(float);
  return (b + 255) & ~(size_t)255;
}
static bool wino_plan(const MfConvDesc* d, MfConvDesc* g, Plan2* pl) {
  if (!wino_shape_ok(d)) return false;
  wino_gemm_desc(d, g);
  if (make_plan2(g, pl) != MF_OK || !pl->ok) return false;
  return pl->splitk == 1 || tree_possible(g, *pl);
}

int mf_wino_ok(const MfConvDesc* d) {
  MfConvDesc g;
  Plan2 pl;
  return wino_plan(d, &g, &pl) ? 1 : 0;
}

struct WinoEntry { int N, H, W, Cin, Cout; };
static const WinoEntry kWinoTable[] = {
#include "wino_plan_table.inc"
    {0, 0, 0, 0, 0},
};
static bool wino_rule(const MfConvDesc* d) {
  const long cin = d->C1 + d->C2, co = d->Cout, hw = (long)d->Hin * d->Win;
  if (cin * co < 190 * (cin + co)) return false;
  if (hw >= 1024 && co >= 512 && cin * co < 300 * (cin + co) && (long)d->N * hw >= 16384) return false;
  return true;
}
int mf_wino_preferred(const MfConvDesc* d) {
  if (!d) return 0;
  static const int mode = [] { const char* e = getenv("MF_WINO_RULE"); return e ? atoi(e) : 1; }();
  if (mode == 0) {
    for (const auto& e : kWinoTable)
      if (e.N == d->N && e.H == d->Hin && e.W == d->Win && e.Cin == d->C1 + d->C2 && e.Cout == d->Cout) return mf_wino_ok(d);
    return 0;
  }
  return wino_rule(d) ? mf_wino_ok(d) : 0;
}
int mf_wino_in_table(const MfConvDesc* d) {
  if (!d) return 0;
  for (const auto& e : kWinoTable)
    if (e.N == d->N && e.H == d->Hin && e.W == d->Win && e.Cin == d->C1 + d->C2 && e.Cout == d->Cout) return 1;
  return 0;
}

size_t mf_wino_workspace_bytes(const MfConvDesc* d) {
  MfConvDesc g;
  Plan2 pl;
  if (!wino_plan(d, &g, &pl)) return 0;
  return wino_m_bytes(d) + (pl.splitk > 1 ? tree_handoff_bytes(&g, pl) : 0);
}

int mf_wino_sync_words(const MfConvDesc* d) {
  MfConvDesc g;
  Plan2 pl;
  if (!wino_plan(d, &g, &pl) || pl.splitk <= 1) return 0;
  return cdiv(pl.M, pl.t.BM) * (g.Cout / pl.t.BN) * (pl.splitk - 1);
}

static int wino_tiles_per_part(const MfConvDesc* d) {
  const int T = (d->Hin / 2) * (d->Win / 2), R = 256 / (d->Cout / 4);
  int parts = T / R;
  if (parts < 1) parts = 1;
  if (parts > 64) parts = 64;
  return cdiv(cdiv(T, parts), R) * R;
}
int mf_wino_gn_parts(const MfConvDesc* d, int G) {
  if (!mf_wino_ok(d) || G <= 0 || G > 256 || d->Cout % G || (d->Cout / G) % 4) return 0;
  return cdiv((d->Hin / 2) * (d->Win / 2), wino_tiles_per_part(d));
}

int mf_wino_pack_weight_f32(const float* w_oihw, float* u, int Cout, int Cin, void* stream) {
  MF_REQUIRE(w_oihw && u && Cout > 0 && Cin > 0, MF_EINVAL, "wino_pack_weight: bad args");
  const long n = (long)Cout * Cin;
  MF_LAUNCH(mfw::wino_pack_weight_kernel, dim3((unsigned)((n + 255) / 256)), dim3(256), 0, (hipStream_t)stream, w_oihw, u, n);
  return check_launch("wino_pack_weight");
}

int mf_wino_input_f16x2(const void* xs, const float* x_bound, void* vs, float* v_bound, int N, int H, int W, int C, void* stream) {
  MF_REQUIRE(xs && vs && N > 0 && H >= 2 && W >= 2 && H % 2 == 0 && W % 2 == 0 && C > 0 && C % 8 == 0, MF_EINVAL,
             "wino_input: bad args (H, W even, C %% 8 == 0)");
  MF_REQUIRE((x_bound == nullptr) == (v_bound == nullptr), MF_EINVAL, "wino_input: x_bound and v_bound go together");
  MF_REQUIRE((double)16 * N * (H / 2) * (W / 2) * C * 4.0 < 4294967040.0, MF_EUNSUPPORTED, "wino_input: the transformed tensor exceeds 4 GB");
  hipStream_t s = (hipStream_t)stream;
  const long total = (long)N * (H / 2) * (W / 2) * (C / 4);
  long blocks = (total + 255) / 256;
  if (blocks > 256 * 16) blocks = 256 * 16;
  const double nelem = (double)N * H * W * C;
  ProfScope ps(MF_FAM_WINO_XFORM, s, 0, 4.0 * nelem * 5.0);
  MF_LAUNCH(mfw::wino_input_kernel, dim3((unsigned)blocks), dim3(256), 0, s, xs, x_bound, vs, v_bound, N, H, W, C);
  return check_launch("wino_input");
}

int mf_conv2d_wino_f16x2(const void* v1s, const void* v2s, const void* us, const float* bias, float* y, const float* v1_bound, const float* v2_bound,
                         float u_bound, void* workspace, size_t workspace_bytes, uint32_t* sync, double* gn_partial, int G, const MfConvDesc* d,
                         void* stream) {
  MF_REQUIRE(d && y && v1s && us && workspace, MF_EINVAL, "conv_wino: null pointer");
  MfConvDesc g;
  Prep q;
  MF_REQUIRE(wino_plan(d, &g, &q.pl), MF_EUNSUPPORTED, "conv_wino: this convolution is not on the Winograd path (ask mf_wino_ok)");
  MF_REQUIRE(!gn_partial || mf_wino_gn_parts(d, G) > 0, MF_EUNSUPPORTED, "conv_wino: cannot emit GroupNorm partials for G = %d (mf_wino_gn_parts == 0)", G);
  const size_t mbytes = wino_m_bytes(d), need = mf_wino_workspace_bytes(d);
  MF_REQUIRE(workspace_bytes >= need, MF_EWORKSPACE, "conv_wino: workspace %zu < %zu", workspace_bytes, need);
  float* m = reinterpret_cast<float*>(workspace);
  int rc = conv_f16x2_prepare(v1s, v2s, us, nullptr, m, v1_bound, v2_bound, u_bound, nullptr, reinterpret_cast<char*>(workspace) + mbytes,
                              workspace_bytes - mbytes, sync, nullptr, 0, nullptr, &g, nullptr, &q, true);
  if (rc) return rc;
  MF_REQUIRE(q.pl.splitk == 1 || q.tree, MF_EUNSUPPORTED, "conv_wino: the component GEMM's split-K must meet inside the launch");
  hipStream_t s = (hipStream_t)stream;
  const int Cin = d->C1 + d->C2, T = (d->Hin / 2) * (d->Win / 2);
  const double M = (double)d->N * d->Hin * d->Win;
  {
    ProfScope ps(MF_FAM_CONV_IGEMM, s, 2.0 * M * d->Cout * 9.0 * Cin, 16.0 * M * Cin + 64.0 * d->Cout * Cin + 16.0 * M * d->Cout, 2.0 * 4.0 * M * d->Cout * Cin * 3.0);
    ps.set_tag(q.pl.t.id, 1);
    rc = dispatch_tile(q.pl.t.id, q.p, s, 3, 0);
    if (rc == -1) { set_error("conv_wino: no tile config %d", q.pl.t.id); rc = MF_EINVAL; }
  }
  if (rc) return rc;
  const int tpp = wino_tiles_per_part(d), parts = cdiv(T, tpp);
  ProfScope ps(MF_FAM_WINO_XFORM, s, 0, 4.0 * M * d->Cout * 5.0);
  MF_LAUNCH(mfw::wino_output_kernel, dim3(parts, d->N), dim3(256), 0, s, (const float*)m, bias, y, gn_partial, d->N, d->Hin, d->Win, d->Cout, G > 0 ? G : 1, tpp);
  return check_launch("wino_output");
}

int mf_wino_tail_ok(const MfConvDesc* d, int G) {
  if (!mf_wino_ok(d) || G <= 0 || d->Cout % G) return 0;
  const int cpg = d->Cout / G;
  if (cpg % 8 || 256 % (cpg / 4)) return 0;
  return (size_t)d->Hin * d->Win * cpg * sizeof(float) <= 64 * 1024 ? 1 : 0;
}

int mf_wino_group_ok(const MfConvDesc* d, const MfConvDesc* guest) {
  static const int off = [] { const char* e = getenv("MF_CONV_GROUP"); return e && atoi(e) == 0 ? 1 : 0; }();
  MfConvDesc g;
  Plan2 pl, pb;
  if (off || !guest || guest->precision != MF_CONV_FP32_F16X2 || !wino_plan(d, &g, &pl)) return 0;
  if (make_plan2(guest, &pb) != MF_OK || !pb.ok || !single_launch(guest, pb, 0)) return 0;
  mfc2::ConvP2 dummy{};
  return dispatch_group(pl.t.id, pb.t.id, dummy, dummy, nullptr, 2) == 1 ? 1 : 0;
}

int mf_conv2d_wino_gn_apply_f16x2(const void* v1s, const void* v2s, const void* us, const float* bias, const float* v1_bound, const float* v2_bound,
                                  float u_bound, void* workspace, size_t workspace_bytes, uint32_t* sync, int G, const MfWinoTail* t,
                                  const MfConvF16x2Call* guest, const MfConvDesc* d, void* stream) {
  MF_REQUIRE(d && t && v1s && us && workspace, MF_EINVAL, "conv_wino_gn_apply: null pointer");
  MF_REQUIRE(mf_wino_tail_ok(d, G), MF_EUNSUPPORTED, "conv_wino_gn_apply: not on this path (mf_wino_tail_ok == 0)");
  MF_REQUIRE(t->out || t->out_split || t->out_wino, MF_EINVAL, "conv_wino_gn_apply: no output");
  MF_REQUIRE(!(t->out_split || t->out_wino) || t->out_bound, MF_EINVAL, "conv_wino_gn_apply: out_bound with the fp16-pair outputs");
  MF_REQUIRE(!t->out_wino || t->wino_bound, MF_EINVAL, "conv_wino_gn_apply: wino_bound with out_wino");
  MF_REQUIRE((t->gamma == nullptr) == (t->beta == nullptr), MF_EINVAL, "conv_wino_gn_apply: gamma/beta must both be given or both NULL");
  MF_REQUIRE(!(t->residual && t->residual_pairs), MF_EINVAL, "conv_wino_gn_apply: the residual is fp32 OR fp16 pairs");
  MF_REQUIRE(!t->residual_pairs || t->res_bound, MF_EINVAL, "conv_wino_gn_apply: a residual given as fp16 pairs needs the res_bound that scaled it");
  MF_REQUIRE(!t->residual || t->res_bound || (t->res_bound_slots && t->res_nslots > 0), MF_EINVAL, "conv_wino_gn_apply: a residual needs res_bound or res_bound_slots");
  MF_REQUIRE(!t->emb || (t->emb_bound && t->emb_stride % 4 == 0), MF_EINVAL, "conv_wino_gn_apply: an embedding needs emb_bound and emb_stride %% 4 == 0");
  MfConvDesc g;
  Prep q;
  MF_REQUIRE(wino_plan(d, &g, &q.pl), MF_EUNSUPPORTED, "conv_wino_gn_apply: not on the Winograd path");
  const size_t mbytes = wino_m_bytes(d), need = mf_wino_workspace_bytes(d);
  MF_REQUIRE(workspace_bytes >= need, MF_EWORKSPACE, "conv_wino_gn_apply: workspace %zu < %zu", workspace_bytes, need);
  float* m = reinterpret_cast<float*>(workspace);
  int rc = conv_f16x2_prepare(v1s, v2s, us, nullptr, m, v1_bound, v2_bound, u_bound, nullptr, reinterpret_cast<char*>(workspace) + mbytes,
                              workspace_bytes - mbytes, sync, nullptr, 0, nullptr, &g, nullptr, &q, true);
  if (rc) return rc;
  MF_REQUIRE(q.pl.splitk == 1 || q.tree, MF_EUNSUPPORTED, "conv_wino_gn_apply: the component GEMM's split-K must meet inside the launch");
  hipStream_t s = (hipStream_t)stream;
  const int Cin = d->C1 + d->C2;
  const double M = (double)d->N * d->Hin * d->Win;
  const double gflops = 2.0 * M * d->Cout * 9.0 * Cin, gbytes = 16.0 * M * Cin + 64.0 * d->Cout * Cin + 16.0 * M * d->Cout , gexec = 2.0 * 4.0 * M * d->Cout * Cin * 3.0;
  if (guest) {
    MF_REQUIRE(guest->d && guest->y && mf_wino_group_ok(d, guest->d), MF_EUNSUPPORTED, "conv_wino_gn_apply: the guest cannot share this launch (mf_wino_group_ok == 0)");
    Prep qb;
    rc = conv_f16x2_prepare(guest->x1s, guest->x2s, guest->ws, guest->bias, guest->y, guest->x1_bound, guest->x2_bound, guest->w_bound, guest->y_bound,
                            guest->workspace, guest->workspace_bytes, guest->sync, guest->gn_partial, guest->G, nullptr, guest->d, nullptr, &qb);
    if (rc) return rc;
    MF_REQUIRE(qb.pl.splitk == 1 || qb.tree, MF_EUNSUPPORTED, "conv_wino_gn_apply: the guest's plan needs its reducer pass");
    if (qb.tree) {
      const char *wa = (const char*)workspace, *wb = (const char*)guest->workspace;
      MF_REQUIRE(wa + need <= wb || wb + tree_handoff_bytes(guest->d, qb.pl) <= wa, MF_EINVAL, "conv_wino_gn_apply: the guest's workspace overlaps the GEMM's");
      const long ca = mf_wino_sync_words(d), cb = mf_conv2d_f16x2_sync_words(guest->d);
      MF_REQUIRE(!sync || sync + ca <= guest->sync || guest->sync + cb <= sync, MF_EINVAL, "conv_wino_gn_apply: the guest's sync array overlaps the GEMM's");
    }
    MF_REQUIRE(guest->y != m, MF_EINVAL, "conv_wino_gn_apply: one output for two convolutions");
    ProfScope ps(MF_FAM_CONV_IGEMM, s, gflops + qb.flops, gbytes + qb.bytes, gexec + 2.0 * 3.0 * qb.pl.M * (double)guest->d->Cout * qb.pl.K);
    ps.set_tag(1000 + 100 * q.pl.t.id + qb.pl.t.id, 1);
    rc = dispatch_group(q.pl.t.id, qb.pl.t.id, q.p, qb.p, s, 0);
    if (rc == -1) { set_error("conv_wino_gn_apply: no tile pair (%d, %d)", q.pl.t.id, qb.pl.t.id); rc = MF_EINVAL; }
  } else {
    ProfScope ps(MF_FAM_CONV_IGEMM, s, gflops, gbytes, gexec);
    ps.set_tag(q.pl.t.id, 1);
    rc = dispatch_tile(q.pl.t.id, q.p, s, 3, 0);
    if (rc == -1) { set_error("conv_wino_gn_apply: no tile config %d", q.pl.t.id); rc = MF_EINVAL; }
  }
  if (rc) return rc;
  mfw::WinoTailP p;
  p.m = m; p.bias = bias; p.gamma = t->gamma; p.beta = t->beta;
  p.res_f32 = t->residual; p.res_pairs = t->residual_pairs; p.res_bound = t->res_bound; p.res_slots = t->res_bound ? nullptr : t->res_bound_slots;
  p.res_nslots = t->res_nslots; p.emb = t->emb; p.emb_stride = (long)t->emb_stride; p.emb_bound = t->emb_bound;
  p.out_f32 = t->out; p.out_pairs = t->out_split; p.out_bound = t->out_bound; p.out_wino = t->out_wino; p.wino_bound = t->wino_bound;
  p.N = d->N; p.H = d->Hin; p.W = d->Win; p.C = d->Cout; p.G = G; p.act = t->act; p.eps = t->eps; p.bconst = t->bconst;
  static const int v_nt = [] { const char* e = getenv("MF_WINO_VSTORE"); return e ? atoi(e) : 1; }();
  p.v_nt = v_nt;
  static const int tail_map = [] { const char* e = getenv("MF_WINO_TAIL_MAP"); return e ? atoi(e) : 1; }();
  p.xcd_map = tail_map;
  p.v_f32 = 0;
  const size_t lds = (size_t)d->Hin * d->Win * (d->Cout / G) * sizeof(float);
  {
    static DeviceOnce once;
    if (first_use_on_device(once)) (void)hipFuncSetAttribute(reinterpret_cast<const void*>(&mfw::wino_tail_kernel), hipFuncAttributeMaxDynamicSharedMemorySize, 64 * 1024);
  }
  ProfScope ps(MF_FAM_WINO_XFORM, s, 8.0 * M * d->Cout, 4.0 * M * d->Cout * (4 + (t->out ? 1 : 0) + (t->out_split ? 1 : 0) + (t->out_wino ? 4 : 0) + (t->residual || t->residual_pairs ? 1 : 0)));
  MF_LAUNCH(mfw::wino_tail_kernel, dim3((unsigned)G * (unsigned)d->N), dim3(256), lds, s, p);
  return check_launch("wino_tail");
}

int mf_wino_f32_ok(const MfConvDesc* d, int G) {
  if (!d || (d->precision != MF_CONV_FP32 && d->precision != MF_CONV_FP32_SPLIT3_W3) || d->KH != 3 || d->KW != 3 || d->stride != 1 || d->pad != 1 || d->upsample != 0 ||
      d->in_layout != MF_LAYOUT_NHWC || d->out_layout != MF_LAYOUT_NHWC || d->N <= 0 || d->Hin < 2 || d->Win < 2 || d->Hin % 2 || d->Win % 2 || d->C1 <= 0 || d->C1 % 32 ||
      d->C2 < 0 || d->C2 % 32 || d->Cout % 64 || d->Cout > 1024 || G <= 0 || d->Cout % G)
    return 0;
  const int cpg = d->Cout / G;
  if (cpg % 4 || 256 % (cpg / 4)) return 0;
  if ((size_t)d->Hin * d->Win * cpg * sizeof(float) > 64 * 1024) return 0;
  const long rows = (long)d->N * (d->Hin / 2) * (d->Win / 2);
  return rows % 64 == 0 && (double)rows * 16.0 < 2147483647.0 ? 1 : 0;
}

int mf_wino_input_f32(const float* x, float* v, int N, int H, int W, int C, void* stream) {
  MF_REQUIRE(x && v && N > 0 && H >= 2 && W >= 2 && H % 2 == 0 && W % 2 == 0 && C > 0 && C % 4 == 0, MF_EINVAL, "wino_input_f32: bad args (H, W even, C %% 4 == 0)");
  hipStream_t s = (hipStream_t)stream;
  const long total = (long)N * (H / 2) * (W / 2) * (C / 4);
  long blocks = (total + 255) / 256;
  if (blocks > 256 * 16) blocks = 256 * 16;
  ProfScope ps(MF_FAM_WINO_XFORM, s, 0, 4.0 * (double)N * H * W * C * 5.0);
  MF_LAUNCH(mfw::wino_input_f32_kernel, dim3((unsigned)blocks), dim3(256), 0, s, x, v, N, H, W, C);
  return check_launch("wino_input_f32");
}

int mf_wino_tail_f32(const float* m, const float* bias, const float* gamma, const float* beta, const float* residual, const float* emb, int64_t emb_stride,
                     float* out, float* out_wino, int N, int H, int W, int C, int G, int act, float eps, void* stream) {
  MF_REQUIRE(m && out && N > 0 && H >= 2 && W >= 2 && H % 2 == 0 && W % 2 == 0 && C > 0 && G > 0 && C % G == 0, MF_EINVAL, "wino_tail_f32: bad args");
  MF_REQUIRE((gamma == nullptr) == (beta == nullptr), MF_EINVAL, "wino_tail_f32: gamma/beta must both be given or both NULL");
  MF_REQUIRE(!emb || emb_stride % 4 == 0, MF_EINVAL, "wino_tail_f32: emb_stride %% 4 == 0");
  const int cpg = C / G;
  MF_REQUIRE(cpg % 4 == 0 && 256 % (cpg / 4) == 0, MF_EUNSUPPORTED, "wino_tail_f32: channels per group %d (a thread keeps its 4 channels)", cpg);
  const size_t lds = (size_t)H * W * cpg * sizeof(float);
  MF_REQUIRE(lds <= 64 * 1024, MF_EUNSUPPORTED, "wino_tail_f32: a sample's pixels x a group's channels do not fit in LDS (%zu bytes)", lds);
  hipStream_t s = (hipStream_t)stream;
  mfw::WinoTailP p;
  p.m = m; p.bias = bias; p.gamma = gamma; p.beta = beta;
  p.res_f32 = residual; p.res_pairs = nullptr; p.res_bound = nullptr; p.res_slots = nullptr; p.res_nslots = 0;
  p.emb = emb; p.emb_stride = (long)emb_stride; p.emb_bound = nullptr;
  p.out_f32 = out; p.out_pairs = nullptr; p.out_bound = nullptr; p.out_wino = out_wino; p.wino_bound = nullptr;
  p.N = N; p.H = H; p.W = W; p.C = C; p.G = G; p.act = act; p.eps = eps; p.bconst = 0.f;
  p.v_nt = 1; p.v_f32 = 1;
  static const int tail_map = [] { const char* e = getenv("MF_WINO_TAIL_MAP"); return e ? atoi(e) : 1; }();
  p.xcd_map = tail_map;
  {
    static DeviceOnce once;
    if (first_use_on_device(once)) (void)hipFuncSetAttribute(reinterpret_cast<const void*>(&mfw::wino_tail_kernel), hipFuncAttributeMaxDynamicSharedMemorySize, 64 * 1024);
  }
  const double M = (double)N * H * W;
  ProfScope ps(MF_FAM_WINO_XFORM, s, 8.0 * M * C, 4.0 * M * C * (4 + 1 + (out_wino ? 4 : 0) + (residual ? 1 : 0)));
  MF_LAUNCH(mfw::wino_tail_kernel, dim3((unsigned)G * (unsigned)N), dim3(256), lds, s, p);
  return check_launch("wino_tail_f32");
}

int mf_wino_plan_query(const MfConvDesc* d, int32_t* tile_id, int32_t* splitk) {
  MfConvDesc g;
  Plan2 pl;
  const bool ok = wino_plan(d, &g, &pl);
  if (tile_id) *tile_id = ok ? pl.t.id : 0;
  if (splitk) *splitk = ok ? pl.splitk : 0;
  return MF_OK;
}
```

### medfusion_amd/csrc/winograd.h

```cpp
#pragma once
#include "common.h"
#include "split_f16.h"

namespace mfw {
using namespace mf;
typedef float wf32x4 __attribute__((ext_vector_type(4)));

__global__ __launch_bounds__(256) void wino_pack_weight_kernel(const float* __restrict__ w, float* __restrict__ u, long n) {
  const long i = (long)blockIdx.x * 256 + threadIdx.x;
  if (i >= n) return;
  double g[3][3], t[4][3];
#pragma unroll
  for (int r = 0; r < 3; ++r)
#pragma unroll
    for (int c = 0; c < 3; ++c) g[r][c] = (double)w[i * 9 + r * 3 + c];
#pragma unroll
  for (int c = 0; c < 3; ++c) {
    t[0][c] = g[0][c];
    t[1][c] = 0.5 * (g[0][c] + g[1][c] + g[2][c]);
    t[2][c] = 0.5 * (g[0][c] - g[1][c] + g[2][c]);
    t[3][c] = g[2][c];
  }
#pragma unroll
  for (int r = 0; r < 4; ++r) {
    const double u0 = t[r][0], u1 = 0.5 * (t[r][0] + t[r][1] + t[r][2]), u2 = 0.5 * (t[r][0] - t[r][1] + t[r][2]), u3 = t[r][2];
    u[(long)(4 * r + 0) * n + i] = (float)u0;
    u[(long)(4 * r + 1) * n + i] = (float)u1;
    u[(long)(4 * r + 2) * n + i] = (float)u2;
    u[(long)(4 * r + 3) * n + i] = (float)u3;
  }
}

__device__ __forceinline__ float4 wino_load_pairs4(const void* pairs, long e) {
  const uint2* g = reinterpret_cast<const uint2*>(reinterpret_cast<const char*>(pairs) + (e >> 3) * 32 + ((e >> 2) & 1) * 8);
  const uint2 h = g[0], l = g[2];
  const sf_f16x2 h0 = __builtin_bit_cast(sf_f16x2, h.x), h1 = __builtin_bit_cast(sf_f16x2, h.y), l0 = __builtin_bit_cast(sf_f16x2, l.x),
                 l1 = __builtin_bit_cast(sf_f16x2, l.y);
  return make_float4((float)h0[0] + (float)l0[0] * kLoInv, (float)h0[1] + (float)l0[1] * kLoInv, (float)h1[0] + (float)l1[0] * kLoInv,
                     (float)h1[1] + (float)l1[1] * kLoInv);
}

__device__ __forceinline__ void wino_bt_d_b(float* d) {
#pragma unroll
  for (int c = 0; c < 4; ++c) {
    const float d0 = d[c], d1 = d[4 + c], d2 = d[8 + c], d3 = d[12 + c];
    d[c] = d0 - d2; d[4 + c] = d1 + d2; d[8 + c] = d2 - d1; d[12 + c] = d1 - d3;
  }
#pragma unroll
  for (int r = 0; r < 4; ++r) {
    const float t0 = d[4 * r], t1 = d[4 * r + 1], t2 = d[4 * r + 2], t3 = d[4 * r + 3];
    d[4 * r] = t0 - t2; d[4 * r + 1] = t1 + t2; d[4 * r + 2] = t2 - t1; d[4 * r + 3] = t1 - t3;
  }
}

__global__ __launch_bounds__(256) void wino_input_kernel(const void* __restrict__ xs, const float* __restrict__ xbound, void* __restrict__ vs,
                                                          float* __restrict__ vbound, int N, int H, int W, int C) {
  const int C4 = C >> 2, TW = W >> 1, T = (H >> 1) * TW;
  const long total = (long)N * T * C4, stride = (long)gridDim.x * 256;
  const long plane = (long)N * T * C;
  for (long i = (long)blockIdx.x * 256 + threadIdx.x; i < total; i += stride) {
    const int c4 = (int)(i % C4);
    const long r = i / C4;
    const int tile = (int)(r % T), n = (int)(r / T);
    const int ty = tile / TW, tx = tile - ty * TW;
    const float b = xbound ? xbound[n] : 0.f;
    const float vb = 4.f * b;
    const float f = xbound ? exp2i(scale_exp_of(b)) * exp2i(-scale_exp_of(vb)) : 1.f;
    float d[4][16];
#pragma unroll
    for (int py = 0; py < 4; ++py)
#pragma unroll
      for (int px = 0; px < 4; ++px) {
        const int y = 2 * ty - 1 + py, x = 2 * tx - 1 + px;
        float4 v = make_float4(0.f, 0.f, 0.f, 0.f);
        if ((unsigned)y < (unsigned)H && (unsigned)x < (unsigned)W) v = wino_load_pairs4(xs, (((long)n * H + y) * W + x) * C + c4 * 4);
        d[0][4 * py + px] = v.x; d[1][4 * py + px] = v.y; d[2][4 * py + px] = v.z; d[3][4 * py + px] = v.w;
      }
#pragma unroll
    for (int k = 0; k < 4; ++k) wino_bt_d_b(d[k]);
    const long e0 = ((long)n * T + tile) * C + c4 * 4;
#pragma unroll
    for (int k = 0; k < 16; ++k) store_split4<true>(vs, (long)k * plane + e0, d[0][k], d[1][k], d[2][k], d[3][k], f);
    if (vbound && tile == 0 && c4 == 0) {
#pragma unroll
      for (int k = 0; k < 16; ++k) vbound[k * N + n] = vb;
    }
  }
}

__global__ __launch_bounds__(256) void wino_input_f32_kernel(const float* __restrict__ x, float* __restrict__ v, int N, int H, int W, int C) {
  const int C4 = C >> 2, TW = W >> 1, T = (H >> 1) * TW;
  const long total = (long)N * T * C4, stride = (long)gridDim.x * 256;
  const long plane = (long)N * T * C;
  for (long i = (long)blockIdx.x * 256 + threadIdx.x; i < total; i += stride) {
    const int c4 = (int)(i % C4);
    const long r = i / C4;
    const int tile = (int)(r % T), n = (int)(r / T);
    const int ty = tile / TW, tx = tile - ty * TW;
    float d[4][16];
#pragma unroll
    for (int py = 0; py < 4; ++py)
#pragma unroll
      for (int px = 0; px < 4; ++px) {
        const int y = 2 * ty - 1 + py, xx = 2 * tx - 1 + px;
        float4 q = make_float4(0.f, 0.f, 0.f, 0.f);
        if ((unsigned)y < (unsigned)H && (unsigned)xx < (unsigned)W) q = *reinterpret_cast<const float4*>(x + (((long)n * H + y) * W + xx) * C + c4 * 4);
        d[0][4 * py + px] = q.x; d[1][4 * py + px] = q.y; d[2][4 * py + px] = q.z; d[3][4 * py + px] = q.w;
      }
#pragma unroll
    for (int k = 0; k < 4; ++k) wino_bt_d_b(d[k]);
    const long e0 = ((long)n * T + tile) * C + c4 * 4;
#pragma unroll
    for (int k = 0; k < 16; ++k) __builtin_nontemporal_store(wf32x4{d[0][k], d[1][k], d[2][k], d[3][k]}, reinterpret_cast<wf32x4*>(v + (long)k * plane + e0));
  }
}

__global__ __launch_bounds__(256) void wino_output_kernel(const float* __restrict__ m, const float* __restrict__ bias, float* __restrict__ y,
                                                           double* __restrict__ gn_partial, int N, int H, int W, int C, int G, int tiles_per_part) {
  __shared__ double sd[2 * 256];
  const int n = blockIdx.y, part = blockIdx.x, parts = gridDim.x, tid = threadIdx.x;
  const int C4 = C >> 2, R = 256 / C4, c4 = tid % C4, tl0 = tid / C4;
  const int TW = W >> 1, T = (H >> 1) * TW;
  const long plane = (long)N * T * C;
  const int t_beg = part * tiles_per_part, t_end = min(T, t_beg + tiles_per_part);
  const float4 b4 = bias ? *reinterpret_cast<const float4*>(bias + c4 * 4) : make_float4(0.f, 0.f, 0.f, 0.f);
  double s = 0, q = 0;
  for (int t = t_beg + tl0; t < t_end; t += R) {
    const float* src = m + ((long)n * T + t) * C + c4 * 4;
    float4 v[16];
#pragma unroll
    for (int k = 0; k < 16; ++k) v[k] = *reinterpret_cast<const float4*>(src + (long)k * plane);
    float4 o[4];
#pragma unroll
    for (int e = 0; e < 4; ++e) {
      float mm[16];
#pragma unroll
      for (int k = 0; k < 16; ++k) mm[k] = e == 0 ? v[k].x : e == 1 ? v[k].y : e == 2 ? v[k].z : v[k].w;
      float a0[4], a1[4];
#pragma unroll
      for (int c = 0; c < 4; ++c) {
        a0[c] = (mm[c] + mm[4 + c]) + mm[8 + c];
        a1[c] = (mm[4 + c] - mm[8 + c]) - mm[12 + c];
      }
      const float be = e == 0 ? b4.x : e == 1 ? b4.y : e == 2 ? b4.z : b4.w;
      const float y00 = ((a0[0] + a0[1]) + a0[2]) + be, y01 = ((a0[1] - a0[2]) - a0[3]) + be;
      const float y10 = ((a1[0] + a1[1]) + a1[2]) + be, y11 = ((a1[1] - a1[2]) - a1[3]) + be;
      if (e == 0) { o[0].x = y00; o[1].x = y01; o[2].x = y10; o[3].x = y11; }
      if (e == 1) { o[0].y = y00; o[1].y = y01; o[2].y = y10; o[3].y = y11; }
      if (e == 2) { o[0].z = y00; o[1].z = y01; o[2].z = y10; o[3].z = y11; }
      if (e == 3) { o[0].w = y00; o[1].w = y01; o[2].w = y10; o[3].w = y11; }
    }
    const int ty = t / TW, tx = t - ty * TW;
    float* dst = y + (((long)n * H + 2 * ty) * W + 2 * tx) * C + c4 * 4;
    *reinterpret_cast<float4*>(dst) = o[0];
    *reinterpret_cast<float4*>(dst + C) = o[1];
    *reinterpret_cast<float4*>(dst + (long)W * C) = o[2];
    *reinterpret_cast<float4*>(dst + (long)W * C + C) = o[3];
    if (gn_partial) {
      float s1 = 0.f, s2 = 0.f;
#pragma unroll
      for (int j = 0; j < 4; ++j) {
        s1 += (o[j].x + o[j].y) + (o[j].z + o[j].w);
        s2 = fmaf(o[j].x, o[j].x, s2); s2 = fmaf(o[j].y, o[j].y, s2); s2 = fmaf(o[j].z, o[j].z, s2); s2 = fmaf(o[j].w, o[j].w, s2);
      }
      s += (double)s1;
      q += (double)s2;
    }
  }
  if (gn_partial) {
    sd[tid] = s;
    sd[256 + tid] = q;
    __syncthreads();
    if (tid < G) {
      const int cq = (C / G) >> 2;
      double a = 0, b = 0;
      for (int tl = 0; tl < R; ++tl)
        for (int k = 0; k < cq; ++k) {
          a += sd[tl * C4 + tid * cq + k];
          b += sd[256 + tl * C4 + tid * cq + k];
        }
      double* o = gn_partial + (((long)n * parts + part) * G + tid) * 2;
      o[0] = a;
      o[1] = b;
// ... 219 lines not shown
```

### medfusion_amd/kernels.py

```python
from __future__ import annotations

import ctypes as C
import os
from typing import Optional

import torch

from . import lib as L


def _gpu(*ts):
    for t in ts:
        if t is None:
            continue
        if not t.is_cuda:
            raise RuntimeError("medfusion_amd: tensors must live on a ROCm device -- the product path has no CPU fallback")
        if t.dtype not in (torch.float32, torch.float64, torch.int64, torch.int32, torch.uint8, torch.int16):
            raise RuntimeError(f"medfusion_amd: unsupported dtype {t.dtype}")


def _ptr(t: Optional[torch.Tensor]) -> Optional[int]:
    return None if t is None else t.data_ptr()


# ... 292 lines not shown


def conv_f16x2_ok(d: L.MfConvDesc) -> bool:
    return bool(L.load().mf_conv2d_f16x2_ok(C.byref(d)))


def conv_plan(d: L.MfConvDesc):
    t, k = C.c_int32(), C.c_int32()
    L.check(L.load().mf_conv2d_plan_query(C.byref(d), C.byref(t), C.byref(k)), "mf_conv2d_plan_query")
    return t.value, k.value


def pin_conv_plan(d: L.MfConvDesc):
    lib = L.load()
    if d.precision in (5, 6) and not (d.tile_hint and d.splitk_hint):
        t, k = conv_plan(d)
        if t > 0 and k > 0:
            d.tile_hint, d.splitk_hint = t, k
    return (lib.mf_conv2d_workspace_bytes(C.byref(d)), (lib.mf_conv2d_f16x2_bound_slots(C.byref(d)) if d.precision in (5, 6) else 0),
            (lib.mf_conv2d_f16x2_sync_words(C.byref(d)) if d.precision in (5, 6) else 0))


def conv2d_f16x2(x1: torch.Tensor, w_split, bias: Optional[torch.Tensor], d: L.MfConvDesc, x2: Optional[torch.Tensor] = None,
                 out: Optional[torch.Tensor] = None, measure_out: bool = False, gn_groups: int = 0, gn_parts: int = 0, pinned=None):
    wh, wmax = w_split
    _gpu(x1, x2, wh, bias)
    lib = L.load()
    x1s, b1 = split_of(x1), bound_of(x1)
    x2s, b2 = (split_of(x2), bound_of(x2)) if x2 is not None else (None, None)
    ho, wo = conv_out_hw(d)
    if out is None:
        out = torch.empty((d.N, ho, wo, d.Cout), dtype=torch.float32, device=x1.device)
    else:
        drop_split(out)
    if pinned is None:
        pinned = (lib.mf_conv2d_workspace_bytes(C.byref(d)), lib.mf_conv2d_f16x2_bound_slots(C.byref(d)) if measure_out and not gn_groups else 0,
                  lib.mf_conv2d_f16x2_sync_words(C.byref(d)))
    need, slots, words = pinned
    if not measure_out or gn_groups:
        slots = 0
    yb = torch.empty((d.N, slots), dtype=torch.float32, device=x1.device) if slots else None
    partial = torch.empty((d.N, gn_parts, gn_groups, 2), dtype=torch.float64, device=x1.device) if gn_groups else None
    ws = Workspace.get(need, x1.device) if need else None
    sync = SyncWords.get(words, x1.device) if words else None
    rc = lib.mf_conv2d_f16x2(x1s.data_ptr(), _ptr(x2s), wh.data_ptr(), _ptr(bias), out.data_ptr(), b1.data_ptr(), _ptr(b2), wmax, _ptr(yb), _ptr(ws), need,
                             _ptr(sync), _ptr(partial), gn_groups, C.byref(d), stream())
    L.check(rc, "mf_conv2d_f16x2")
    if slots:
        out._mf_slots = yb
        _stamp(out)
    return (out, partial) if gn_groups else out


def conv_group_ok(da: L.MfConvDesc, Ga: int, db: L.MfConvDesc, Gb: int) -> bool:
    return bool(L.load().mf_conv2d_f16x2_group_ok(C.byref(da), Ga, C.byref(db), Gb))


def conv2d_f16x2_group(x1: torch.Tensor, x2: Optional[torch.Tensor], a, b):
    _gpu(x1, x2, a["w_split"][0], b["w_split"][0], a["bias"], b["bias"])
    lib = L.load()
    dev = x1.device
    x1s, b1 = split_of(x1), bound_of(x1)
    x2s, b2 = (split_of(x2), bound_of(x2)) if x2 is not None else (None, None)
    da, db = a["d"], b["d"]
    need_a, _, words_a = a["pinned"]
    need_b, slots_b, words_b = b["pinned"]
    off_b = (need_a + 255) & ~255
    ws = Workspace.get(off_b + need_b, dev) if (need_a or need_b) else None
    sync = SyncWords.get(words_a + words_b, dev) if (words_a or words_b) else None
    hoa, woa = conv_out_hw(da)
    hob, wob = conv_out_hw(db)
    ya = torch.empty((da.N, hoa, woa, da.Cout), dtype=torch.float32, device=dev)
    yb = torch.empty((db.N, hob, wob, db.Cout), dtype=torch.float32, device=dev)
    G, parts = a["gn_groups"], a["gn_parts"]
    partial = torch.empty((da.N, parts, G, 2), dtype=torch.float64, device=dev)
    slots = torch.empty((db.N, slots_b), dtype=torch.float32, device=dev) if slots_b else None
    (wa, wmax_a), (wb, wmax_b) = a["w_split"], b["w_split"]
    ca = L.MfConvF16x2Call(x1s.data_ptr(), _ptr(x2s), wa.data_ptr(), _ptr(a["bias"]), ya.data_ptr(), b1.data_ptr(), _ptr(b2), wmax_a, None,
                           ws.data_ptr() if need_a else None, need_a, sync.data_ptr() if words_a else None, partial.data_ptr(), G, C.pointer(da))
    cb = L.MfConvF16x2Call(x1s.data_ptr(), _ptr(x2s), wb.data_ptr(), _ptr(b["bias"]), yb.data_ptr(), b1.data_ptr(), _ptr(b2), wmax_b, _ptr(slots),
                           ws.data_ptr() + off_b if need_b else None, need_b, sync.data_ptr() + 4 * words_a if words_b else None, None, 0, C.pointer(db))
    L.check(lib.mf_conv2d_f16x2_group(C.byref(ca), C.byref(cb), stream()), "mf_conv2d_f16x2_group")
    if slots_b:
        yb._mf_slots = slots
        _stamp(yb)
    return (ya, partial), yb


def pack_nchw_pairs(x_nchw: torch.Tensor, cp: int = 32) -> torch.Tensor:
    _gpu(x_nchw)
    x = x_nchw.contiguous()
    n, c, h, w = x.shape
    out = torch.empty((n, h, w, cp), dtype=torch.float32, device=x.device)
    outs = torch.empty((n, h, w, cp), dtype=torch.int32, device=x.device)
    ob = torch.empty((n,), dtype=torch.float32, device=x.device)
    L.check(L.load().mf_pack_nchw_pairs_f32(x.data_ptr(), outs.data_ptr(), ob.data_ptr(), n, c, h * w, cp, stream()), "mf_pack_nchw_pairs_f32")
    out._mf_split, out._mf_bound, out._mf_pairs_only = outs, ob, True
    _stamp(out)
    _audit(out, "pack_nchw_pairs (measured)")
    return out


def conv_pairs_out_ok(d: L.MfConvDesc) -> bool:
    return bool(L.load().mf_conv2d_f16x2_pairs_out_ok(C.byref(d)))


def conv2d_f16x2_pairs_out(x1: torch.Tensor, w_split, bias: Optional[torch.Tensor], d: L.MfConvDesc, l1, bias_max: float, x2: Optional[torch.Tensor] = None,
                           pinned=None) -> torch.Tensor:
    wh, wmax = w_split
    _gpu(x1, x2, wh, bias)
    lib = L.load()
    x1s, b1 = split_of(x1), bound_of(x1)
    x2s, b2 = (split_of(x2), bound_of(x2)) if x2 is not None else (None, None)
    ho, wo = conv_out_hw(d)
    out = torch.empty((d.N, ho, wo, d.Cout), dtype=torch.float32, device=x1.device)
    outs = torch.empty((d.N, ho, wo, d.Cout), dtype=torch.int32, device=x1.device)
    ob = torch.empty((d.N,), dtype=torch.float32, device=x1.device)
    if pinned is None:
        pinned = (lib.mf_conv2d_workspace_bytes(C.byref(d)), 0, lib.mf_conv2d_f16x2_sync_words(C.byref(d)))
    need, _, words = pinned
    ws = Workspace.get(need, x1.device) if need else None
    sync = SyncWords.get(words, x1.device) if words else None
    rc = lib.mf_conv2d_f16x2_pairs_out(x1s.data_ptr(), _ptr(x2s), wh.data_ptr(), _ptr(bias), out.data_ptr(), outs.data_ptr(), ob.data_ptr(), b1.data_ptr(), _ptr(b2),
                                       wmax, float(l1[0]), float(l1[1]), float(bias_max), _ptr(ws), need, _ptr(sync), C.byref(d), stream())
    L.check(rc, "mf_conv2d_f16x2_pairs_out")
    out._mf_split, out._mf_bound = outs, ob
    _stamp(out)
    _audit(out, "conv pairs_out (derived: bound(x) L1(w) + max|bias|)")
    return out


def wino_ok(d: L.MfConvDesc) -> bool:
    return bool(L.load().mf_wino_ok(C.byref(d)))


def wino_preferred(d: L.MfConvDesc) -> bool:
    return bool(L.load().mf_wino_preferred(C.byref(d)))


def wino_gn_parts(d: L.MfConvDesc, G: int) -> int:
    return L.load().mf_wino_gn_parts(C.byref(d), G)


def wino_pack_weight(w_oihw: torch.Tensor) -> torch.Tensor:
    _gpu(w_oihw)
    w = w_oihw.contiguous()
    co, ci, kh, kw = w.shape
    assert (kh, kw) == (3, 3)
    out = torch.empty((16, co, 1, 1, ci), dtype=torch.float32, device=w.device)
    L.check(L.load().mf_wino_pack_weight_f32(w.data_ptr(), out.data_ptr(), co, ci, stream()), "mf_wino_pack_weight_f32")
    return out


def wino_input(x: torch.Tensor):
    v = _fresh(x, "_mf_wino")
    if v is None:
        site = getattr(x, "_mf_wino_site", None)
        if site is not None:
            site[0][site[1]] = True
        xs, xb = split_of(x), bound_of(x)
        n, h, w, c = x.shape
        v = torch.empty((16, n, (h // 2) * (w // 2), c), dtype=torch.int32, device=x.device)
        vb = torch.empty((16 * n,), dtype=torch.float32, device=x.device)
        L.check(L.load().mf_wino_input_f16x2(xs.data_ptr(), xb.data_ptr(), v.data_ptr(), vb.data_ptr(), n, h, w, c, stream()), "mf_wino_input_f16x2")
        x._mf_wino, x._mf_wino_bound = v, vb
        _stamp(x)
    return v, x._mf_wino_bound


def pin_wino_plan(d: L.MfConvDesc):
    lib = L.load()
    return lib.mf_wino_workspace_bytes(C.byref(d)), lib.mf_wino_sync_words(C.byref(d))


def conv2d_wino_f16x2(x1: torch.Tensor, u_split, bias: Optional[torch.Tensor], d: L.MfConvDesc, x2: Optional[torch.Tensor] = None,
                      gn_groups: int = 0, gn_parts: int = 0, pinned=None):
    uh, umax = u_split
    _gpu(x1, x2, uh, bias)
    lib = L.load()
    v1, b1 = wino_input(x1)
    v2, b2 = wino_input(x2) if x2 is not None else (None, None)
    dev = x1.device
    out = torch.empty((d.N, d.Hin, d.Win, d.Cout), dtype=torch.float32, device=dev)
    partial = torch.empty((d.N, gn_parts, gn_groups, 2), dtype=torch.float64, device=dev) if gn_groups else None
    need, words = pinned if pinned is not None else pin_wino_plan(d)
    ws = Workspace.get(need, dev)
    sync = SyncWords.get(words, dev) if words else None
    rc = lib.mf_conv2d_wino_f16x2(v1.data_ptr(), _ptr(v2), uh.data_ptr(), _ptr(bias), out.data_ptr(), b1.data_ptr(), _ptr(b2), umax, ws.data_ptr(), need,
                                  _ptr(sync), _ptr(partial), gn_groups, C.byref(d), stream())
    L.check(rc, "mf_conv2d_wino_f16x2")
    return (out, partial) if gn_groups else out


def wino_tail_ok(d: L.MfConvDesc, G: int) -> bool:
    return bool(L.load().mf_wino_tail_ok(C.byref(d), G))


def wino_group_ok(d: L.MfConvDesc, guest: L.MfConvDesc) -> bool:
    return bool(L.load().mf_wino_group_ok(C.byref(d), C.byref(guest)))


def conv2d_wino_gn_apply(x1: torch.Tensor, u_split, bias: Optional[torch.Tensor], d: L.MfConvDesc, gamma, beta, G: int, eps: float, act: int = 1,
                         residual: Optional[torch.Tensor] = None, emb: Optional[torch.Tensor] = None, emb_stride: int = 0,
                         x2: Optional[torch.Tensor] = None, bconst: float = 0.0, out_fp32: bool = True, want_wino: bool = False, pinned=None,
                         guest=None) -> torch.Tensor:
    uh, umax = u_split
    _gpu(x1, x2, uh, bias, gamma, beta, residual, emb)
    lib = L.load()
    v1, b1 = wino_input(x1)
    v2, b2 = wino_input(x2) if x2 is not None else (None, None)
    n, h, w, c = d.N, d.Hin, d.Win, d.Cout
    dev = x1.device
    need, words = pinned if pinned is not None else pin_wino_plan(d)
    gcall = None
    if guest is not None:
        if residual is not None:
            raise RuntimeError("conv2d_wino_gn_apply: the guest's output is the residual")
        dg = guest["d"]
        need_g, slots_g, words_g = guest["pinned"]
        off_g = (need + 255) & ~255
        ws = Workspace.get(off_g + need_g, dev)
        sync = SyncWords.get(words + words_g, dev) if (words or words_g) else None
        x1s, xb1 = split_of(x1), bound_of(x1)
        x2s, xb2 = (split_of(x2), bound_of(x2)) if x2 is not None else (None, None)
        hog, wog = conv_out_hw(dg)
        residual = torch.empty((dg.N, hog, wog, dg.Cout), dtype=torch.float32, device=dev)
        gslots = torch.empty((dg.N, slots_g), dtype=torch.float32, device=dev) if slots_g else None
        wg, wgmax = guest["w_split"]
        gcall = L.MfConvF16x2Call(x1s.data_ptr(), _ptr(x2s), wg.data_ptr(), _ptr(guest["bias"]), residual.data_ptr(), xb1.data_ptr(), _ptr(xb2), wgmax, _ptr(gslots),
                                  ws.data_ptr() + off_g if need_g else None, need_g, sync.data_ptr() + 4 * words if words_g else None, None, 0, C.pointer(dg))
        if slots_g:
            residual._mf_slots = gslots
            _stamp(residual)
    else:
        ws = Workspace.get(need, dev)
        sync = SyncWords.get(words, dev) if words else None
    res_pairs = rb = rslots = eb = None
    if residual is not None:
        if pairs_only(residual):
            res_pairs, rb = residual._mf_split, residual._mf_bound
        elif _fresh(residual, "_mf_bound") is None and _fresh(residual, "_mf_slots") is not None:
            rslots = residual._mf_slots
        else:
            rb = bound_of(residual)
    if emb is not None:
        eb = _fresh(emb, "_mf_bound")
        if eb is None:
            eb = maxabs_rows(emb.contiguous())
    out = torch.empty((n, h, w, c), dtype=torch.float32, device=dev)
    outs = torch.empty((n, h, w, c), dtype=torch.int32, device=dev)
    ob = torch.empty((n,), dtype=torch.float32, device=dev)
    ov = torch.empty((16, n, (h // 2) * (w // 2), c), dtype=torch.int32, device=dev) if want_wino else None
    ovb = torch.empty((16 * n,), dtype=torch.float32, device=dev) if want_wino else None
    t = L.MfWinoTail(_ptr(gamma), _ptr(beta), None if res_pairs is not None else _ptr(residual), _ptr(res_pairs), _ptr(rb), _ptr(rslots), _ptr(emb), _ptr(eb),
                     out.data_ptr() if out_fp32 else None, outs.data_ptr(), ob.data_ptr(), _ptr(ov), _ptr(ovb), int(emb_stride),
                     0 if rslots is None else rslots.shape[1], int(act), float(bconst), float(eps))
    rc = lib.mf_conv2d_wino_gn_apply_f16x2(v1.data_ptr(), _ptr(v2), uh.data_ptr(), _ptr(bias), b1.data_ptr(), _ptr(b2), umax, ws.data_ptr(), need, _ptr(sync), G,
                                           C.byref(t), None if gcall is None else C.byref(gcall), C.byref(d), stream())
    L.check(rc, "mf_conv2d_wino_gn_apply_f16x2")
    out._mf_split, out._mf_bound = outs, ob
    if want_wino:
        out._mf_wino, out._mf_wino_bound = ov, ovb
    _stamp(out)
    _audit(out, "Winograd tail (derived: bconst + residual + embedding)")
    if not out_fp32:
        out._mf_pairs_only = True
    return out


def wino_f32_ok(d: L.MfConvDesc, G: int) -> bool:
    return bool(L.load().mf_wino_f32_ok(C.byref(d), G))


def wino_input_f32(x: torch.Tensor) -> torch.Tensor:
    v = _fresh(x, "_mf_wino_f32")
    if v is None:
        _need_f32(x)
        site = getattr(x, "_mf_wino_site_f32", None)
        if site is not None:
            site[0][site[1]] = True
        n, h, w, c = x.shape
        v = torch.empty((16, n, (h // 2) * (w // 2), c), dtype=torch.float32, device=x.device)
        L.check(L.load().mf_wino_input_f32(x.data_ptr(), v.data_ptr(), n, h, w, c, stream()), "mf_wino_input_f32")
        x._mf_wino_f32 = v
        _stamp(x)
    return v


def conv2d_wino_gn_apply_f32(x1: torch.Tensor, u_packed: torch.Tensor, bias: Optional[torch.Tensor], d: L.MfConvDesc, gamma, beta, G: int, eps: float,
                             act: int = 1, residual: Optional[torch.Tensor] = None, emb: Optional[torch.Tensor] = None, emb_stride: int = 0,
                             x2: Optional[torch.Tensor] = None, want_wino: bool = False) -> torch.Tensor:
    _gpu(x1, x2, u_packed, bias, gamma, beta, residual, emb)
    lib = L.load()
    n, h, w, c1 = x1.shape
    c2 = 0 if x2 is None else x2.shape[-1]
    co, t = d.Cout, (h // 2) * (w // 2)
    v1 = wino_input_f32(x1)
    v2 = wino_input_f32(x2) if x2 is not None else None
    g = make_conv_desc(16 * n, 1, t, c1, c2, co, 1, 1, 0, 3, precision=d.precision)
    m = conv2d(v1.view(16 * n, 1, t, c1), u_packed, None, g, x2=None if v2 is None else v2.view(16 * n, 1, t, c2))
    assert m.numel() == 16 * n * t * co, (tuple(m.shape), n, t, co)
    if residual is not None:
        _need_f32(residual)
    out = torch.empty((n, h, w, co), dtype=torch.float32, device=x1.device)
    ov = torch.empty((16, n, t, co), dtype=torch.float32, device=x1.device) if want_wino else None
    L.check(lib.mf_wino_tail_f32(m.data_ptr(), _ptr(bias), _ptr(gamma), _ptr(beta), _ptr(residual), _ptr(emb), emb_stride, out.data_ptr(), _ptr(ov),
                                 n, h, w, co, G, act, eps, stream()), "mf_wino_tail_f32")
    if want_wino:
        out._mf_wino_f32 = ov
        _stamp(out)
    return out


def conv_fuse_words(d: L.MfConvDesc, G: int) -> int:
    return L.load().mf_conv2d_f16x2_fuse_words(C.byref(d), G)


def conv2d_f16x2_gn_apply(x1: torch.Tensor, w_split, bias: Optional[torch.Tensor], d: L.MfConvDesc, gamma, beta, G: int, eps: float, parts: int,
                          words: int, act: int = 1, residual: Optional[torch.Tensor] = None, emb: Optional[torch.Tensor] = None, emb_stride: int = 0,
                          x2: Optional[torch.Tensor] = None, bconst: float = 0.0, out_fp32: bool = True, pinned=None) -> torch.Tensor:
    wh, wmax = w_split
    _gpu(x1, x2, wh, bias, gamma, beta, residual, emb)
    lib = L.load()
    x1s, b1 = split_of(x1), bound_of(x1)
    x2s, b2 = (split_of(x2), bound_of(x2)) if x2 is not None else (None, None)
    ho, wo = conv_out_hw(d)
    n, c = d.N, d.Cout
    dev = x1.device
    res_pairs = rb = rslots = eb = None
    if residual is not None:
        if pairs_only(residual):
            res_pairs, rb = residual._mf_split, residual._mf_bound
        elif _fresh(residual, "_mf_bound") is None and _fresh(residual, "_mf_slots") is not None:
            rslots = residual._mf_slots
        else:
            rb = bound_of(residual)
    if emb is not None:
        eb = _fresh(emb, "_mf_bound")
        if eb is None:
            eb = maxabs_rows(emb.contiguous())
    out = torch.empty((n, ho, wo, c), dtype=torch.float32, device=dev)
    outs = torch.empty((n, ho, wo, c), dtype=torch.int32, device=dev)
    ob = torch.empty((n,), dtype=torch.float32, device=dev)
    partial = torch.empty((n, parts, G, 2), dtype=torch.float64, device=dev)
    if pinned is None:
        pinned = (lib.mf_conv2d_workspace_bytes(C.byref(d)), 0, lib.mf_conv2d_f16x2_sync_words(C.byref(d)))
    need, _, swords = pinned
    ws = Workspace.get(need, dev) if need else None
    sync = SyncWords.get(swords, dev) if swords else None
    rv = Rendezvous.get(words, dev)
    f = L.MfGnFuse(_ptr(gamma), _ptr(beta), None if res_pairs is not None else _ptr(residual), _ptr(res_pairs), _ptr(rb), _ptr(rslots), _ptr(emb), _ptr(eb),
                   out.data_ptr() if out_fp32 else None, outs.data_ptr(), ob.data_ptr(), rv.data_ptr() + 16, rv.data_ptr(), int(emb_stride),
                   0 if rslots is None else rslots.shape[1], int(act), float(bconst), float(eps))
    rc = lib.mf_conv2d_f16x2_gn_apply(x1s.data_ptr(), _ptr(x2s), wh.data_ptr(), _ptr(bias), b1.data_ptr(), _ptr(b2), wmax, _ptr(ws), need, _ptr(sync),
                                      partial.data_ptr(), G, C.byref(f), C.byref(d), stream())
    L.check(rc, "mf_conv2d_f16x2_gn_apply")
    out._mf_split, out._mf_bound = outs, ob
    _stamp(out)
    _audit(out, "conv + GroupNorm tail in one launch (derived)")
    if not out_fp32:
        out._mf_pairs_only = True
    return out


def make_conv3d_desc(N, D, H, W, C1, C2, Cout, k, stride=(1, 1, 1), pad=(0, 0, 0), upsample=(0, 0, 0), tile_hint=0, splitk_hint=0,
                     precision=5) -> L.MfConv3dDesc:
    t3 = lambda v: (int(v),) * 3 if isinstance(v, int) else tuple(int(a) for a in v)
    A = C.c_int32 * 3
    return L.MfConv3dDesc(N, D, H, W, C1, C2, Cout, k, A(*t3(stride)), A(*t3(pad)), A(*t3(upsample)), tile_hint, splitk_hint, precision)


def conv3d_ok(d: L.MfConv3dDesc) -> bool:
    return bool(L.load().mf_conv3d_ok(C.byref(d)))


def conv3d_out_dims(d: L.MfConv3dDesc):
    out = (C.c_int32 * 3)()
    L.check(L.load().mf_conv3d_out_dims(C.byref(d), out), "mf_conv3d_out_dims")
    return tuple(out)


def conv3d_plan(d: L.MfConv3dDesc):
    t, k = C.c_int32(), C.c_int32()
    L.check(L.load().mf_conv3d_plan_query(C.byref(d), C.byref(t), C.byref(k)), "mf_conv3d_plan_query")
    return t.value, k.value


def pack_conv3d_weight(w_oidhw: torch.Tensor, cin_pad: int = 0) -> torch.Tensor:
    _gpu(w_oidhw)
    w = w_oidhw.detach().contiguous()
    co, ci, k = w.shape[0], w.shape[1], w.shape[2]
    if w.dim() != 5 or tuple(w.shape[2:]) != (k, k, k):
        raise RuntimeError(f"pack_conv3d_weight: OIDHW weights with a cubic kernel, got {tuple(w.shape)}")
    cp = cin_pad or ci
    out = torch.empty((co, k, k, k, cp), dtype=torch.float32, device=w.device)
    L.check(L.load().mf_pack_conv3d_weight_f32(w.data_ptr(), out.data_ptr(), co, ci, k, cp, stream()), "mf_pack_conv3d_weight_f32")
    return out


def conv3d_f16x2(x1: torch.Tensor, w_split, bias: Optional[torch.Tensor], d: L.MfConv3dDesc, x2: Optional[torch.Tensor] = None,
                 out: Optional[torch.Tensor] = None) -> torch.Tensor:
    wh, wmax = w_split
    _gpu(x1, x2, wh, bias)
    lib = L.load()
    if not lib.mf_conv3d_ok(C.byref(d)):
        raise RuntimeError("conv3d_f16x2: descriptor not supported (mf_conv3d_ok)")
    x1s, b1 = split_of(x1), bound_of(x1)
    x2s, b2 = (split_of(x2), bound_of(x2)) if x2 is not None else (None, None)
    do, ho, wo = conv3d_out_dims(d)
    if out is None:
        out = torch.empty((d.N, do, ho, wo, d.Cout), dtype=torch.float32, device=x1.device)
    else:
# ... 570 lines not shown
```

### medfusion_amd/lib.py

```python
from __future__ import annotations

import ctypes as C
import os
from pathlib import Path

HERE = Path(__file__).resolve().parent
LIB_PATH = HERE / "libmedfusion_hip.so"

c_fp = C.c_void_p


class MfConvDesc(C.Structure):
    _fields_ = [(n, C.c_int32) for n in (
        "N", "Hin", "Win", "C1", "C2", "Cout", "KH", "KW", "stride", "pad", "upsample", "in_layout", "out_layout",
        "tile_hint", "splitk_hint", "precision")]


class MfConv3dDesc(C.Structure):
    _fields_ = ([(n, C.c_int32) for n in ("N", "D", "H", "W", "C1", "C2", "Cout", "k")] + [(n, C.c_int32 * 3) for n in ("stride", "pad", "upsample")]
                + [(n, C.c_int32) for n in ("tile_hint", "splitk_hint", "precision")])


class MfSchedStep(C.Structure):
    _fields_ = [("sqrt_recip_ac", C.c_float), ("sqrt_recipm1_ac", C.c_float), ("coef1", C.c_float), ("coef2", C.c_float),
                ("std_fixed", C.c_float), ("log_var_min", C.c_float), ("log_var_max", C.c_float), ("ddim_sqrt_an", C.c_float),
                ("ddim_c", C.c_float), ("ddim_sigma", C.c_float), ("t", C.c_int32), ("mode", C.c_int32)]


class MfSchedArgs(C.Structure):
    _fields_ = [("x_t", c_fp), ("pred", c_fp), ("pred_uncond", c_fp), ("pred_var", c_fp), ("noise_post", c_fp), ("noise_ddim", c_fp),
                ("noise_step_stride", C.c_int64), ("x_t_out", c_fp), ("x0_out", c_fp), ("xT_out", c_fp), ("table", c_fp),
                ("step_dev", c_fp), ("step", C.c_int32), ("objective", C.c_int32), ("clip_x0", C.c_int32),
                ("guidance_scale", C.c_float), ("n", C.c_int64)]


class MfSchedBlend(C.Structure):
    _fields_ = [("z0", c_fp), ("eps0", c_fp), ("mask", c_fp), ("coef", c_fp), ("cells", C.c_int64), ("channels", C.c_int32), ("reserved", C.c_int32)]


SOLVER_FINAL, SOLVER_DDIM0, SOLVER_ORDER1, SOLVER_ORDER2 = 0, 1, 2, 3


class MfSolverStep(C.Structure):
    _fields_ = [("sqrt_recip_ac", C.c_float), ("sqrt_recipm1_ac", C.c_float), ("A", C.c_float), ("B", C.c_float), ("C", C.c_float), ("t", C.c_int32),
                ("mode", C.c_int32), ("reserved", C.c_int32)]


class MfSolverArgs(C.Structure):
    _fields_ = [("x_t", c_fp), ("pred", c_fp), ("pred_uncond", c_fp), ("x_t_out", c_fp), ("x0_out", c_fp), ("xT_out", c_fp), ("x0_hist", c_fp),
                ("table", c_fp), ("step_counter", c_fp), ("ticket", c_fp), ("step_dev", c_fp), ("step", C.c_int32), ("objective", C.c_int32),
                ("clip_x0", C.c_int32), ("guidance_scale", C.c_float), ("n", C.c_int64)]


class MfGnFuse(C.Structure):
    _fields_ = [("gamma", c_fp), ("beta", c_fp), ("residual", c_fp), ("residual_pairs", c_fp), ("res_bound", c_fp), ("res_bound_slots", c_fp),
                ("emb", c_fp), ("emb_bound", c_fp), ("out", c_fp), ("out_split", c_fp), ("out_bound", c_fp), ("rendezvous", c_fp), ("error_flag", c_fp),
                ("emb_stride", C.c_int64), ("res_nslots", C.c_int32), ("act", C.c_int32), ("bconst", C.c_float), ("eps", C.c_float)]


class MfWinoTail(C.Structure):
    _fields_ = [("gamma", c_fp), ("beta", c_fp), ("residual", c_fp), ("residual_pairs", c_fp), ("res_bound", c_fp), ("res_bound_slots", c_fp),
                ("emb", c_fp), ("emb_bound", c_fp), ("out", c_fp), ("out_split", c_fp), ("out_bound", c_fp), ("out_wino", c_fp), ("wino_bound", c_fp),
                ("emb_stride", C.c_int64), ("res_nslots", C.c_int32), ("act", C.c_int32), ("bconst", C.c_float), ("eps", C.c_float)]


class MfProfRow(C.Structure):
    _fields_ = [("tag", C.c_int32), ("variant", C.c_int32), ("launches", C.c_int64), ("ms", C.c_double), ("flops", C.c_double), ("bytes", C.c_double),
                ("exec_flops", C.c_double)]


class MfConvF16x2Call(C.Structure):
    _fields_ = [("x1s", c_fp), ("x2s", c_fp), ("ws", c_fp), ("bias", c_fp), ("y", c_fp), ("x1_bound", c_fp), ("x2_bound", c_fp), ("w_bound", C.c_float),
                ("y_bound", c_fp), ("workspace", c_fp), ("workspace_bytes", C.c_size_t), ("sync", c_fp), ("gn_partial", c_fp), ("G", C.c_int32),
                ("d", C.POINTER(MfConvDesc))]


LAYOUT_NHWC, LAYOUT_NCHW = 0, 1
FAMILIES = ("conv_igemm", "conv_direct", "splitk_reduce", "gn_stats", "gn_apply", "linear", "sched", "noise", "attention", "misc", "conv_gn_fused", "wino_xform")

_I, _I64, _F, _SZ, _U64 = C.c_int, C.c_int64, C.c_float, C.c_size_t, C.c_uint64
_SIGS = {
    "mf_version": (C.c_int, []),
    "mf_last_error": (C.c_char_p, []),
    "mf_pack_conv_weight_f32": (_I, [c_fp, c_fp, _I, _I, _I, _I, c_fp]),
    "mf_pack_upconv_weight_f32": (_I, [c_fp, c_fp, _I, _I, c_fp]),
    "mf_conv2d_subpixel_ok": (_I, [C.POINTER(MfConvDesc)]),
    "mf_conv2d_is_igemm": (_I, [C.POINTER(MfConvDesc)]),
    "mf_split_conv_weight_bf16x3": (_I, [c_fp, c_fp, C.c_long, _I, c_fp]),
    "mf_convert_conv_weight_bf16": (_I, [c_fp, c_fp, C.c_long, _I, c_fp]),
    "mf_conv2d_workspace_bytes": (_SZ, [C.POINTER(MfConvDesc)]),
    "mf_conv2d_f16x2_ok": (_I, [C.POINTER(MfConvDesc)]),
    "mf_split_f16x2": (_I, [c_fp, c_fp, c_fp, _I, _I64, c_fp]),
    "mf_split_f16x2_slots": (_I, [c_fp, c_fp, c_fp, _I, c_fp, _I, _I64, c_fp]),
    "mf_conv2d_f16x2": (_I, [c_fp, c_fp, c_fp, c_fp, c_fp, c_fp, c_fp, _F, c_fp, c_fp, _SZ, c_fp, c_fp, _I, C.POINTER(MfConvDesc), c_fp]),
    "mf_conv2d_f16x2_sync_words": (_I, [C.POINTER(MfConvDesc)]),
    "mf_pack_nchw_pairs_f32": (_I, [c_fp, c_fp, c_fp, _I, _I, _I, _I, c_fp]),
    "mf_conv2d_f16x2_pairs_out_ok": (_I, [C.POINTER(MfConvDesc)]),
    "mf_conv2d_f16x2_pairs_out": (_I, [c_fp, c_fp, c_fp, c_fp, c_fp, c_fp, c_fp, c_fp, c_fp, _F, _F, _F, _F, c_fp, _SZ, c_fp, C.POINTER(MfConvDesc), c_fp]),
    "mf_conv2d_f16x2_fuse_words": (_I, [C.POINTER(MfConvDesc), _I]),
    "mf_conv2d_f16x2_gn_apply": (_I, [c_fp, c_fp, c_fp, c_fp, c_fp, c_fp, _F, c_fp, _SZ, c_fp, c_fp, _I, C.POINTER(MfGnFuse), C.POINTER(MfConvDesc), c_fp]),
    "mf_conv2d_f16x2_group_ok": (_I, [C.POINTER(MfConvDesc), _I, C.POINTER(MfConvDesc), _I]),
    "mf_conv2d_f16x2_group": (_I, [C.POINTER(MfConvF16x2Call), C.POINTER(MfConvF16x2Call), c_fp]),
    "mf_wino_ok": (_I, [C.POINTER(MfConvDesc)]),
    "mf_wino_preferred": (_I, [C.POINTER(MfConvDesc)]),
    "mf_wino_in_table": (_I, [C.POINTER(MfConvDesc)]),
    "mf_wino_pack_weight_f32": (_I, [c_fp, c_fp, _I, _I, c_fp]),
    "mf_wino_input_f16x2": (_I, [c_fp, c_fp, c_fp, c_fp, _I, _I, _I, _I, c_fp]),
    "mf_wino_workspace_bytes": (_SZ, [C.POINTER(MfConvDesc)]),
    "mf_wino_sync_words": (_I, [C.POINTER(MfConvDesc)]),
    "mf_wino_gn_parts": (_I, [C.POINTER(MfConvDesc), _I]),
    "mf_wino_plan_query": (_I, [C.POINTER(MfConvDesc), C.POINTER(C.c_int32), C.POINTER(C.c_int32)]),
    "mf_wino_f32_ok": (_I, [C.POINTER(MfConvDesc), _I]),
    "mf_wino_input_f32": (_I, [c_fp, c_fp, _I, _I, _I, _I, c_fp]),
    "mf_wino_tail_f32": (_I, [c_fp, c_fp, c_fp, c_fp, c_fp, c_fp, _I64, c_fp, c_fp, _I, _I, _I, _I, _I, _I, _F, c_fp]),
    "mf_conv2d_wino_f16x2": (_I, [c_fp, c_fp, c_fp, c_fp, c_fp, c_fp, c_fp, _F, c_fp, _SZ, c_fp, c_fp, _I, C.POINTER(MfConvDesc), c_fp]),
    "mf_wino_tail_ok": (_I, [C.POINTER(MfConvDesc), _I]),
    "mf_wino_group_ok": (_I, [C.POINTER(MfConvDesc), C.POINTER(MfConvDesc)]),
    "mf_conv2d_wino_gn_apply_f16x2": (_I, [c_fp, c_fp, c_fp, c_fp, c_fp, c_fp, _F, c_fp, _SZ, c_fp, _I, C.POINTER(MfWinoTail), C.POINTER(MfConvF16x2Call),
                                           C.POINTER(MfConvDesc), c_fp]),
    "mf_maxabs_rows_slots": (_I, [_I64]),
    "mf_maxabs_rows_f32": (_I, [c_fp, c_fp, c_fp, _I, _I64, c_fp]),
    "mf_bound_finalize_f32": (_I, [c_fp, c_fp, _I, _I, c_fp]),
    "mf_conv2d_f16x2_bound_slots": (_I, [C.POINTER(MfConvDesc)]),
    "mf_conv2d_plan_override": (_I, [C.POINTER(MfConvDesc), _I, _I]),
    "mf_conv2d_plan_query": (_I, [C.POINTER(MfConvDesc), C.POINTER(C.c_int32), C.POINTER(C.c_int32)]),
    "mf_gn_apply_split_f32": (_I, [c_fp, c_fp, c_fp, c_fp, c_fp, c_fp, _I64, c_fp, c_fp, c_fp, c_fp, c_fp, _F, c_fp, _I, _I, _I, _I, _I, c_fp]),
    "mf_gn_apply_from_partials_f32": (_I, [c_fp, c_fp, _I, _F, c_fp, c_fp, c_fp, c_fp, _I64, c_fp, c_fp, c_fp, c_fp, _I, c_fp, _F, c_fp, _I, _I, _I, _I, _I, c_fp]),
    "mf_gn_apply_from_partials_pairs_f32": (_I, [c_fp, c_fp, _I, _F, c_fp, c_fp, c_fp, c_fp, c_fp, _I64, c_fp, c_fp, c_fp, c_fp, _I, c_fp, _F, c_fp, _I, _I, _I, _I, _I, c_fp]),
    "mf_conv2d_f32": (_I, [c_fp, c_fp, c_fp, c_fp, c_fp, c_fp, _SZ, C.POINTER(MfConvDesc), c_fp]),
    "mf_conv2d_gn_parts": (_I, [C.POINTER(MfConvDesc), _I]),
    "mf_conv2d_gn_f32": (_I, [c_fp, c_fp, c_fp, c_fp, c_fp, c_fp, _SZ, c_fp, _I, C.POINTER(MfConvDesc), c_fp]),
    "mf_gn_partial_parts": (_I, [_I]),
    "mf_gn_finalize_f32": (_I, [c_fp, _I, c_fp, _I, _I, _I, _I, _F, c_fp]),
    "mf_gn_stats_partial_f32": (_I, [c_fp, c_fp, _I, _I, _I, _I, c_fp]),
    "mf_gn_stats_workspace_bytes": (_SZ, [_I, _I, _I, _I]),
    "mf_gn_stats_f32": (_I, [c_fp, c_fp, c_fp, _SZ, _I, _I, _I, _I, _F, c_fp]),
    "mf_gn_apply_f32": (_I, [c_fp, c_fp, c_fp, c_fp, c_fp, c_fp, _I64, c_fp, _I, _I, _I, _I, _I, c_fp]),
    "mf_linear_f32": (_I, [c_fp, _I64, c_fp, c_fp, c_fp, _I64, _I, _I, _I, _I, _I, _I, c_fp]),
    "mf_sinusoidal_f32": (_I, [c_fp, c_fp, c_fp, _I, _I, _F, _F, _I, c_fp]),
    "mf_learned_sinusoidal_f32": (_I, [c_fp, c_fp, c_fp, _I, _I, c_fp]),
    "mf_embedding_add_f32": (_I, [c_fp, c_fp, c_fp, _I, _I, _I, c_fp]),
    "mf_sched_step_f32": (_I, [C.POINTER(MfSchedArgs), c_fp]),
    "mf_sched_step_philox_f32": (_I, [C.POINTER(MfSchedArgs), _U64, C.c_int32, C.c_int32, _I64, _I, c_fp, c_fp, c_fp]),
    "mf_sched_step_blend_f32": (_I, [C.POINTER(MfSchedArgs), C.POINTER(MfSchedBlend), c_fp]),
    "mf_sched_step_philox_blend_f32": (_I, [C.POINTER(MfSchedArgs), _U64, C.c_int32, C.c_int32, _I64, _I, c_fp, c_fp, C.POINTER(MfSchedBlend), c_fp]),
    "mf_solver_step_f32": (_I, [C.POINTER(MfSolverArgs), c_fp]),
    "mf_solver_step_blend_f32": (_I, [C.POINTER(MfSolverArgs), C.POINTER(MfSchedBlend), c_fp]),
    "mf_select_cells_f32": (_I, [c_fp, c_fp, c_fp, c_fp, _I, _I, _I64, c_fp]),
    "mf_mask_maxpool_u8": (_I, [c_fp, _I, c_fp, _I, _I, _I, _I, _I, _I, _I, c_fp]),
    "mf_image_ingress_u8": (_I, [c_fp, c_fp, _I, _I, _I, _I, c_fp]),
    "mf_gather_step_rows3_f32": (_I, [C.POINTER(c_fp), C.POINTER(_I64), C.POINTER(c_fp), _I, c_fp, c_fp, C.c_int32, _I, _I, c_fp]),
    "mf_broadcast_from_table_f32": (_I, [c_fp, c_fp, C.c_int32, c_fp, _I, c_fp]),
    "mf_gather_step_rows_f32": (_I, [c_fp, c_fp, c_fp, C.c_int32, _I, _I64, c_fp, _I, c_fp]),
    "mf_rows_axpby_f32": (_I, [c_fp, c_fp, c_fp, c_fp, c_fp, c_fp, _I, _I64, _I, _F, _F, c_fp]),
    "mf_image_egress_u8": (_I, [c_fp, c_fp, c_fp, _I, _I, _I, _I, _I, c_fp]),
    "mf_avgpool2d_nhwc_f32": (_I, [c_fp, c_fp, _I, _I, _I, _I, _I, _I, _I, c_fp]),
    "mf_upsample_nearest2x_nhwc_f32": (_I, [c_fp, c_fp, _I, _I, _I, _I, c_fp]),
    "mf_pixel_unshuffle2_add_nhwc_f32": (_I, [c_fp, c_fp, _I, _I, _I, _I, c_fp]),
    "mf_pixel_shuffle2_add_nhwc_f32": (_I, [c_fp, c_fp, _I, _I, _I, _I, c_fp]),
    "mf_counter_add_i32": (_I, [c_fp, C.c_int32, c_fp]),
    "mf_philox_normal_f32": (_I, [c_fp, _U64, C.c_int32, C.c_int32, c_fp, C.c_int32, _I64, _I, _I64, c_fp]),
    "mf_attention_f32": (_I, [c_fp, c_fp, c_fp, c_fp, _I, _I, _I, _I, _I, _F, c_fp]),
    "mf_layernorm_f32": (_I, [c_fp, c_fp, c_fp, c_fp, _I64, _I, _F, c_fp]),
    "mf_geglu_f32": (_I, [c_fp, c_fp, _I64, _I, c_fp]),
    "mf_add_f32": (_I, [c_fp, c_fp, c_fp, _I64, c_fp]),
    "mf_nchw_to_nhwc_f32": (_I, [c_fp, c_fp, _I, _I, _I, _I, c_fp]),
    "mf_nhwc_to_nchw_f32": (_I, [c_fp, c_fp, _I, _I, _I, _I, c_fp]),
    "mf_diag_gaussian_sample_f32": (_I, [c_fp, c_fp, c_fp, _I, _I, _I, c_fp]),
    "mf_diag_gaussian_kl_f32": (_I, [c_fp, c_fp, _I, _I, _I, c_fp]),
    "mf_vq_workspace_bytes": (_SZ, [_I64]),
    "mf_vector_quantize_f32": (_I, [c_fp, c_fp, c_fp, c_fp, c_fp, c_fp, _SZ, _I, _I, _I, _I, c_fp]),
    "mf_conv3d_ok": (_I, [C.POINTER(MfConv3dDesc)]),
    "mf_conv3d_out_dims": (_I, [C.POINTER(MfConv3dDesc), C.POINTER(C.c_int32)]),
    "mf_conv3d_plan_query": (_I, [C.POINTER(MfConv3dDesc), C.POINTER(C.c_int32), C.POINTER(C.c_int32)]),
    "mf_conv3d_workspace_bytes": (_SZ, [C.POINTER(MfConv3dDesc)]),
    "mf_pack_conv3d_weight_f32": (_I, [c_fp, c_fp, _I, _I, _I, _I, c_fp]),
    "mf_conv3d_f16x2": (_I, [c_fp, c_fp, c_fp, c_fp, c_fp, c_fp, c_fp, _F, c_fp, _SZ, C.POINTER(MfConv3dDesc), c_fp]),
    "mf_prof_enable": (_I, [_I]),
    "mf_prof_reset": (_I, []),
    "mf_prof_query": (_I, [_I, C.POINTER(C.c_double), C.POINTER(_I64), C.POINTER(C.c_double), C.POINTER(C.c_double)]),
    "mf_prof_query2": (_I, [_I, C.POINTER(C.c_double), C.POINTER(_I64), C.POINTER(C.c_double), C.POINTER(C.c_double), C.POINTER(C.c_double)]),
    "mf_prof_family_name": (C.c_char_p, [_I]),
    "mf_prof_rows": (_I, [_I, C.POINTER(MfProfRow), _I]),
    "mf_prof_tag_name": (_I, [_I, _I, C.c_char_p, _I]),
    "mf_mfma_rate_probe_f16": (_I, [c_fp, c_fp, _I, _I, C.POINTER(C.c_double), c_fp]),
    "mf_cmdlist_begin": (_I, []),
    "mf_cmdlist_end": (_I, [C.POINTER(C.c_void_p)]),
    "mf_cmdlist_count": (_I, [c_fp]),
    "mf_cmdlist_replay": (_I, [c_fp, _I, c_fp]),
    "mf_cmdlist_free": (_I, [c_fp]),
}

_lib = None


def load(build_if_missing: bool = True) -> C.CDLL:
    global _lib
    if _lib is not None:
        return _lib
    path = LIB_PATH
    override = os.environ.get("MEDFUSION_LIB")
    if override:
        path = Path(override)
        if not path.exists():
            raise RuntimeError(f"MEDFUSION_LIB={override}: no such file")
    elif build_if_missing:
        try:
            import fcntl

            from . import build as _build

            with open(str(LIB_PATH) + ".lock", "w") as lock:
                fcntl.flock(lock, fcntl.LOCK_EX)
                if _build.needs_build():
                    _build.build(verbose=bool(os.environ.get("MEDFUSION_VERBOSE_BUILD")))
        except Exception as e:
            if not LIB_PATH.exists():
                raise RuntimeError(f"libmedfusion_hip.so is missing and could not be built: {e}") from e
    if not path.exists():
        raise RuntimeError(f"{path} not found: build it with `python -m medfusion_amd.build` (hipcc, gfx950)")
    lib = C.CDLL(str(path))
    for name, (res, args) in _SIGS.items():
        fn = getattr(lib, name)
        fn.restype, fn.argtypes = res, args
    _lib = lib
    return lib


def last_error() -> str:
    return load().mf_last_error().decode(errors="replace")


def check(rc: int, what: str) -> None:
    if rc != 0:
        raise RuntimeError(f"{what} failed (code {rc}): {last_error()}")


def exported_symbols():
    return sorted(_SIGS)
```

Baseline: 41.45.

## Add panel-tiled Winograd weight layout option and skip pixel decode for wino GEMM

```diff
diff --git a/include/medfusion_hip.h b/include/medfusion_hip.h
--- a/include/medfusion_hip.h
+++ b/include/medfusion_hip.h
@@ -126,6 +126,16 @@
 int mf_conv2d_wino_gn_apply_f16x2(const void* v1s, const void* v2s, const void* us, const float* bias, const float* v1_bound, const float* v2_bound,
                                   float u_bound, void* workspace, size_t workspace_bytes, uint32_t* sync, int G, const MfWinoTail* t,
                                   const MfConvF16x2Call* guest, const MfConvDesc* d, void* stream);
+enum { MF_WINO_U_ROWMAJOR = 0, MF_WINO_U_PANELS = 1 };
+int mf_wino_upanel_default(void);
+size_t mf_wino_tile_weight_bytes(int Cout, int Cin);
+int mf_wino_tile_weight_f16x2(const void* us, void* us_panels, int Cout, int Cin, void* stream);
+int mf_conv2d_wino_f16x2_l(const void* v1s, const void* v2s, const void* us, int u_layout, const float* bias, float* y, const float* v1_bound,
+                           const float* v2_bound, float u_bound, void* workspace, size_t workspace_bytes, uint32_t* sync, double* gn_partial, int G,
+                           const MfConvDesc* d, void* stream);
+int mf_conv2d_wino_gn_apply_f16x2_l(const void* v1s, const void* v2s, const void* us, int u_layout, const float* bias, const float* v1_bound,
+                                    const float* v2_bound, float u_bound, void* workspace, size_t workspace_bytes, uint32_t* sync, int G,
+                                    const MfWinoTail* t, const MfConvF16x2Call* guest, const MfConvDesc* d, void* stream);
 
 int mf_conv2d_gn_parts(const MfConvDesc* d, int G);
 int mf_conv2d_gn_f32(const float* x1, const float* x2, const float* w_packed, const float* bias, float* y, void* workspace,
diff --git a/medfusion_amd/blocks.py b/medfusion_amd/blocks.py
--- a/medfusion_amd/blocks.py
+++ b/medfusion_amd/blocks.py
@@ -39,6 +39,7 @@
         self._wb = None
         self._wh = None
         self._wu = None
+        self._wu_panel = False
         self._l1 = {}
         self._subpixel = subpixel
 
@@ -62,8 +63,11 @@
 
     def get_wino(self, weight: torch.Tensor):
         self.get(weight)
-        if self._wu is None:
+        if self._wu is None or self._wu_panel != wino_upanel():
+            self._wu_panel = wino_upanel()
             self._wu = K.split_weight_f16x2(K.wino_pack_weight(self._raw))
+            if self._wu_panel:
+                self._wu = K.wino_tile_weight(self._wu)
         return self._wu
 
     def get_wino_f32(self, weight: torch.Tensor, split3: bool):
@@ -118,6 +122,16 @@
 WINOGRAD_F32_MFMA = int(os.environ.get("MEDFUSION_WINOGRAD_F32_MFMA", "0"))
 WINO_TAIL = os.environ.get("MEDFUSION_WINOGRAD_TAIL", "1") != "0"
 WINO_GROUP = os.environ.get("MEDFUSION_WINOGRAD_GROUP", "1") != "0"
+WINO_UPANEL = None
+
+
+def wino_upanel() -> bool:
+    global WINO_UPANEL
+    if WINO_UPANEL is None:
+        WINO_UPANEL = K.wino_upanel_default()
+    return bool(WINO_UPANEL)
+
+
 WINO_SHAPES = {}
 if os.environ.get("MEDFUSION_WINOGRAD_TABLE"):
     import json as _json
diff --git a/medfusion_amd/csrc/conv_f16x2.h b/medfusion_amd/csrc/conv_f16x2.h
--- a/medfusion_amd/csrc/conv_f16x2.h
+++ b/medfusion_amd/csrc/conv_f16x2.h
@@ -61,6 +61,7 @@
   int subpix, hw_src;
   int out_nt;
   int wphase_rows;
+  int wpanel;
   int walk_n_fast;
   double* gn_partial;
   int gn_groups, gn_parts, gn_cpg;
diff --git a/medfusion_amd/csrc/conv_f16x2.hip b/medfusion_amd/csrc/conv_f16x2.hip
--- a/medfusion_amd/csrc/conv_f16x2.hip
+++ b/medfusion_amd/csrc/conv_f16x2.hip
@@ -481,7 +481,7 @@
 struct Prep { mfc2::ConvP2 p; Plan2 pl; bool tree; double flops, bytes; int terms; };
 static int conv_f16x2_prepare(const void* x1s, const void* x2s, const void* ws, const float* bias, float* y, const float* x1_bound, const float* x2_bound,
                               float w_bound, float* y_bound, void* workspace, size_t workspace_bytes, uint32_t* sync, double* gn_partial, int G,
-                              const MfGnFuse* fz, const MfConvDesc* d, const PairsOut* po, Prep* out, bool wino_gemm = false) {
+                              const MfGnFuse* fz, const MfConvDesc* d, const PairsOut* po, Prep* out, bool wino_gemm = false, int u_layout = 0) {
   MF_REQUIRE(d && pair_precision(d->precision), MF_EINVAL, "conv(f16x2): desc.precision must be MF_CONV_FP32_F16X2 (or the opt-in MF_CONV_F16)");
   MF_REQUIRE((d->upsample == 3) == wino_gemm, MF_EINVAL, "conv(f16x2): upsample = 3 is internal to mf_conv2d_wino_f16x2");
   Plan2& pl = out->pl;
@@ -508,7 +508,11 @@
   p.bytes1 = (unsigned)(4.0 * d->N * d->Hin * d->Win * d->C1);
   p.bytes2 = (unsigned)(4.0 * d->N * d->Hin * d->Win * d->C2);
   p.bytesw = (unsigned)(4.0 * d->Cout * pl.K * (p.subpix ? 4 : wino_gemm ? 16 : 1));
+#ifdef MFC2_WPITCH_PAD
+  if (wino_gemm) p.bytesw = (unsigned)(16.0 * d->Cout * (4.0 * pl.K + (MFC2_WPITCH_PAD)));
+#endif
   p.wphase_rows = wino_gemm ? (d->N / 16) * d->Hin * d->Win : 0;
+  p.wpanel = wino_gemm && u_layout == MF_WINO_U_PANELS ? 1 : 0;
   {
     static const int walk = [] { const char* e = getenv("MF_CONV_WALK"); return e ? atoi(e) : 1; }();
     const double act_bytes = 4.0 * d->N * d->Hin * d->Win * (d->C1 + d->C2), w_bytes = 4.0 * d->Cout * pl.K * (p.subpix ? 4 : 1);
diff --git a/medfusion_amd/csrc/conv_f16x2_body.inc b/medfusion_amd/csrc/conv_f16x2_body.inc
--- a/medfusion_amd/csrc/conv_f16x2_body.inc
+++ b/medfusion_amd/csrc/conv_f16x2_body.inc
@@ -67,6 +67,11 @@
 #pragma unroll
   for (int i = 0; i < GP; ++i) {
     const int m = m0 + 8 * (wave + NW * i) + lrow;
+    if (p.wphase_rows) {
+      a_pix[i] = m;
+      a_inv[i] = m < p.M ? ~1 : ~0;
+      continue;
+    }
     int n_ = 0, iy0 = -(1 << 28), ix0 = 0;
     if (m < p.M) {
       const int n = qdiv(m, p.HWout, r_hw);
@@ -95,8 +100,13 @@
   }
   const __amdgpu_buffer_rsrc_t rsw = __builtin_amdgcn_make_buffer_rsrc(const_cast<void*>(p.w), 0, p.bytesw, 0x00020000);
   const int phase_t = p.subpix ? ((m0 % p.HWout) / p.hw_src) : (p.wphase_rows ? m0 / p.wphase_rows : 0);
+#ifdef MFC2_WPITCH_PAD
+  const unsigned kbytes = (unsigned)p.K * 4u + (p.wphase_rows ? (unsigned)(MFC2_WPITCH_PAD) : 0u);
+#else
   const unsigned kbytes = (unsigned)p.K * 4u;
-  const unsigned qv = (unsigned)(phase_t * p.Cout + n0 + 8 * wave + lrow) * kbytes + slot16;
+#endif
+  const unsigned wrowb = p.wpanel ? 128u : kbytes, wcs = p.wpanel ? 256u : 4u;
+  const unsigned qv = (unsigned)(phase_t * p.Cout + n0) * kbytes + (unsigned)(8 * wave + lrow) * wrowb + slot16;
 
   int l_cc = cg_beg, l_ky = 0, l_kx = 0, l_it = 0, l_st = 0;
   unsigned pbase[GP], l_off[GP];
@@ -118,7 +128,7 @@
     const unsigned ts_ = (unsigned)(l_ky * p.KW + l_kx);                                                                \
     const unsigned tapb_ = (unsigned)(l_ky * p.Win + l_kx) * l_cs4;                                                     \
     _Pragma("unroll") for (int i = 0; i < GP; ++i) l_off[i] = (pbase[i] + tapb_) | (unsigned)__builtin_amdgcn_sbfe(a_inv[i], ts_, 1u); \
-    l_so = (ts_ * (unsigned)p.Cin + (unsigned)l_cc * 32u) * 4u;                                                         \
+    l_so = (ts_ * (unsigned)p.Cin + (unsigned)l_cc * 32u) * wcs;                                                        \
     l_lds = l_st * STAGE + wave * 1024;                                                                                 \
   }
 #define MFC2_LOAD_UNIT(U)                                                                                               \
@@ -130,7 +140,7 @@
     } else {                                                                                                            \
       constexpr int q_ = u_ - GP;                                                                                       \
       __builtin_amdgcn_raw_ptr_buffer_load_lds(rsw, (__attribute__((address_space(3))) void*)(smem + l_lds + BM * ROWB + NW * q_ * 1024), 16, qv, \
-                                               l_so + (unsigned)q_ * (8u * NW) * kbytes, 0, 0);                         \
+                                               l_so + (unsigned)(q_ * 8 * NW / 64 * 64) * kbytes + (unsigned)(q_ * 8 * NW % 64) * wrowb, 0, 0); \
     }                                                                                                                   \
   }
 #define MFC2_LOAD_ADVANCE()                  \
diff --git a/medfusion_amd/csrc/conv_f16x2_wino.inc b/medfusion_amd/csrc/conv_f16x2_wino.inc
--- a/medfusion_amd/csrc/conv_f16x2_wino.inc
+++ b/medfusion_amd/csrc/conv_f16x2_wino.inc
@@ -93,6 +93,26 @@
   return check_launch("wino_pack_weight");
 }
 
+#ifndef MF_WINO_UPANEL_DEFAULT
+#define MF_WINO_UPANEL_DEFAULT 0
+#endif
+int mf_wino_upanel_default(void) {
+  static const int on = [] { const char* e = getenv("MF_WINO_UPANEL"); return e ? (atoi(e) != 0 ? 1 : 0) : MF_WINO_UPANEL_DEFAULT; }();
+  return on;
+}
+size_t mf_wino_tile_weight_bytes(int Cout, int Cin) {
+  if (Cout <= 0 || Cin <= 0 || Cin % 32) return 0;
+  return (size_t)16 * ((Cout + 63) / 64 * 64) * Cin * 4;
+}
+int mf_wino_tile_weight_f16x2(const void* us, void* us_panels, int Cout, int Cin, void* stream) {
+  MF_REQUIRE(us && us_panels && us != us_panels && Cout > 0 && Cin > 0 && Cin % 32 == 0, MF_EINVAL, "wino_tile_weight: bad args (Cin %% 32 == 0, out of place)");
+  const long slots = (long)(mf_wino_tile_weight_bytes(Cout, Cin) / 16);
+  MF_REQUIRE(slots < (1L << 31) * 256, MF_EUNSUPPORTED, "wino_tile_weight: too large");
+  MF_LAUNCH(mfw::wino_tile_weight_kernel, dim3((unsigned)((slots + 255) / 256)), dim3(256), 0, (hipStream_t)stream, reinterpret_cast<const uint4*>(us),
+            reinterpret_cast<uint4*>(us_panels), Cout, Cin / 32, slots);
+  return check_launch("wino_tile_weight");
+}
+
 int mf_wino_input_f16x2(const void* xs, const float* x_bound, void* vs, float* v_bound, int N, int H, int W, int C, void* stream) {
   MF_REQUIRE(xs && vs && N > 0 && H >= 2 && W >= 2 && H % 2 == 0 && W % 2 == 0 && C > 0 && C % 8 == 0, MF_EINVAL,
              "wino_input: bad args (H, W even, C %% 8 == 0)");
@@ -111,7 +131,13 @@
 int mf_conv2d_wino_f16x2(const void* v1s, const void* v2s, const void* us, const float* bias, float* y, const float* v1_bound, const float* v2_bound,
                          float u_bound, void* workspace, size_t workspace_bytes, uint32_t* sync, double* gn_partial, int G, const MfConvDesc* d,
                          void* stream) {
+  return mf_conv2d_wino_f16x2_l(v1s, v2s, us, MF_WINO_U_ROWMAJOR, bias, y, v1_bound, v2_bound, u_bound, workspace, workspace_bytes, sync, gn_partial, G, d, stream);
+}
+int mf_conv2d_wino_f16x2_l(const void* v1s, const void* v2s, const void* us, int u_layout, const float* bias, float* y, const float* v1_bound,
+                           const float* v2_bound, float u_bound, void* workspace, size_t workspace_bytes, uint32_t* sync, double* gn_partial, int G,
+                           const MfConvDesc* d, void* stream) {
   MF_REQUIRE(d && y && v1s && us && workspace, MF_EINVAL, "conv_wino: null pointer");
+  MF_REQUIRE(u_layout == MF_WINO_U_ROWMAJOR || u_layout == MF_WINO_U_PANELS, MF_EINVAL, "conv_wino: u_layout %d", u_layout);
   MfConvDesc g;
   Prep q;
   MF_REQUIRE(wino_plan(d, &g, &q.pl), MF_EUNSUPPORTED, "conv_wino: this convolution is not on the Winograd path (ask mf_wino_ok)");
@@ -120,7 +146,7 @@
   MF_REQUIRE(workspace_bytes >= need, MF_EWORKSPACE, "conv_wino: workspace %zu < %zu", workspace_bytes, need);
   float* m = reinterpret_cast<float*>(workspace);
   int rc = conv_f16x2_prepare(v1s, v2s, us, nullptr, m, v1_bound, v2_bound, u_bound, nullptr, reinterpret_cast<char*>(workspace) + mbytes,
-                              workspace_bytes - mbytes, sync, nullptr, 0, nullptr, &g, nullptr, &q, true);
+                              workspace_bytes - mbytes, sync, nullptr, 0, nullptr, &g, nullptr, &q, true, u_layout);
   if (rc) return rc;
   MF_REQUIRE(q.pl.splitk == 1 || q.tree, MF_EUNSUPPORTED, "conv_wino: the component GEMM's split-K must meet inside the launch");
   hipStream_t s = (hipStream_t)stream;
@@ -159,7 +185,13 @@
 int mf_conv2d_wino_gn_apply_f16x2(const void* v1s, const void* v2s, const void* us, const float* bias, const float* v1_bound, const float* v2_bound,
                                   float u_bound, void* workspace, size_t workspace_bytes, uint32_t* sync, int G, const MfWinoTail* t,
                                   const MfConvF16x2Call* guest, const MfConvDesc* d, void* stream) {
+  return mf_conv2d_wino_gn_apply_f16x2_l(v1s, v2s, us, MF_WINO_U_ROWMAJOR, bias, v1_bound, v2_bound, u_bound, workspace, workspace_bytes, sync, G, t, guest, d, stream);
+}
+int mf_conv2d_wino_gn_apply_f16x2_l(const void* v1s, const void* v2s, const void* us, int u_layout, const float* bias, const float* v1_bound,
+                                    const float* v2_bound, float u_bound, void* workspace, size_t workspace_bytes, uint32_t* sync, int G,
+                                    const MfWinoTail* t, const MfConvF16x2Call* guest, const MfConvDesc* d, void* stream) {
   MF_REQUIRE(d && t && v1s && us && workspace, MF_EINVAL, "conv_wino_gn_apply: null pointer");
+  MF_REQUIRE(u_layout == MF_WINO_U_ROWMAJOR || u_layout == MF_WINO_U_PANELS, MF_EINVAL, "conv_wino_gn_apply: u_layout %d", u_layout);
   MF_REQUIRE(mf_wino_tail_ok(d, G), MF_EUNSUPPORTED, "conv_wino_gn_apply: not on this path (mf_wino_tail_ok == 0)");
   MF_REQUIRE(t->out || t->out_split || t->out_wino, MF_EINVAL, "conv_wino_gn_apply: no output");
   MF_REQUIRE(!(t->out_split || t->out_wino) || t->out_bound, MF_EINVAL, "conv_wino_gn_apply: out_bound with the fp16-pair outputs");
@@ -176,7 +208,7 @@
   MF_REQUIRE(workspace_bytes >= need, MF_EWORKSPACE, "conv_wino_gn_apply: workspace %zu < %zu", workspace_bytes, need);
   float* m = reinterpret_cast<float*>(workspace);
   int rc = conv_f16x2_prepare(v1s, v2s, us, nullptr, m, v1_bound, v2_bound, u_bound, nullptr, reinterpret_cast<char*>(workspace) + mbytes,
-                              workspace_bytes - mbytes, sync, nullptr, 0, nullptr, &g, nullptr, &q, true);
+                              workspace_bytes - mbytes, sync, nullptr, 0, nullptr, &g, nullptr, &q, true, u_layout);
   if (rc) return rc;
   MF_REQUIRE(q.pl.splitk == 1 || q.tree, MF_EUNSUPPORTED, "conv_wino_gn_apply: the component GEMM's split-K must meet inside the launch");
   hipStream_t s = (hipStream_t)stream;
diff --git a/medfusion_amd/csrc/winograd.h b/medfusion_amd/csrc/winograd.h
--- a/medfusion_amd/csrc/winograd.h
+++ b/medfusion_amd/csrc/winograd.h
@@ -29,6 +29,19 @@
     u[(long)(4 * r + 2) * n + i] = (float)u2;
     u[(long)(4 * r + 3) * n + i] = (float)u3;
   }
+}
+
+__global__ __launch_bounds__(256) void wino_tile_weight_kernel(const uint4* __restrict__ us, uint4* __restrict__ up, int Cout, int chunks, long slots) {
+  const long i = (long)blockIdx.x * 256 + threadIdx.x;
+  if (i >= slots) return;
+  const int s = (int)(i & 7), rr = (int)((i >> 3) & 63);
+  const long pc = i >> 9;
+  const int c = (int)(pc % chunks), npan = (Cout + 63) / 64;
+  const long kp = pc / chunks;
+  const int k = (int)(kp / npan), r = (int)(kp % npan) * 64 + rr;
+  uint4 v = make_uint4(0u, 0u, 0u, 0u);
+  if (r < Cout) v = us[(((long)k * Cout + r) * chunks + c) * 8 + s];
+  up[i] = v;
 }
 
 __device__ __forceinline__ float4 wino_load_pairs4(const void* pairs, long e) {
diff --git a/medfusion_amd/kernels.py b/medfusion_amd/kernels.py
--- a/medfusion_amd/kernels.py
+++ b/medfusion_amd/kernels.py
@@ -468,6 +468,26 @@
     return out
 
 
+def wino_upanel_default() -> bool:
+    return bool(L.load().mf_wino_upanel_default())
+
+
+def wino_tile_weight(u_split):
+    uh, umax = u_split
+    _gpu(uh)
+    co, ci = uh.shape[1], uh.shape[-1]
+    cop = (co + 63) // 64 * 64
+    assert L.load().mf_wino_tile_weight_bytes(co, ci) == 16 * cop * ci * 4
+    up = torch.empty((16, cop // 64, ci // 32, 64, 32), dtype=torch.int32, device=uh.device)
+    L.check(L.load().mf_wino_tile_weight_f16x2(uh.data_ptr(), up.data_ptr(), co, ci, stream()), "mf_wino_tile_weight_f16x2")
+    up._mf_upanel = True
+    return up, umax
+
+
+def _u_layout(uh: torch.Tensor) -> int:
+    return 1 if getattr(uh, "_mf_upanel", False) else 0
+
+
 def wino_input(x: torch.Tensor):
     v = _fresh(x, "_mf_wino")
     if v is None:
@@ -502,9 +522,9 @@
     need, words = pinned if pinned is not None else pin_wino_plan(d)
     ws = Workspace.get(need, dev)
     sync = SyncWords.get(words, dev) if words else None
-    rc = lib.mf_conv2d_wino_f16x2(v1.data_ptr(), _ptr(v2), uh.data_ptr(), _ptr(bias), out.data_ptr(), b1.data_ptr(), _ptr(b2), umax, ws.data_ptr(), need,
+    rc = lib.mf_conv2d_wino_f16x2_l(v1.data_ptr(), _ptr(v2), uh.data_ptr(), _u_layout(uh), _ptr(bias), out.data_ptr(), b1.data_ptr(), _ptr(b2), umax, ws.data_ptr(), need,
                                   _ptr(sync), _ptr(partial), gn_groups, C.byref(d), stream())
-    L.check(rc, "mf_conv2d_wino_f16x2")
+    L.check(rc, "mf_conv2d_wino_f16x2_l")
     return (out, partial) if gn_groups else out
 
 
@@ -571,9 +591,9 @@
     t = L.MfWinoTail(_ptr(gamma), _ptr(beta), None if res_pairs is not None else _ptr(residual), _ptr(res_pairs), _ptr(rb), _ptr(rslots), _ptr(emb), _ptr(eb),
                      out.data_ptr() if out_fp32 else None, outs.data_ptr(), ob.data_ptr(), _ptr(ov), _ptr(ovb), int(emb_stride),
                      0 if rslots is None else rslots.shape[1], int(act), float(bconst), float(eps))
-    rc = lib.mf_conv2d_wino_gn_apply_f16x2(v1.data_ptr(), _ptr(v2), uh.data_ptr(), _ptr(bias), b1.data_ptr(), _ptr(b2), umax, ws.data_ptr(), need, _ptr(sync), G,
-                                           C.byref(t), None if gcall is None else C.byref(gcall), C.byref(d), stream())
-    L.check(rc, "mf_conv2d_wino_gn_apply_f16x2")
+    rc = lib.mf_conv2d_wino_gn_apply_f16x2_l(v1.data_ptr(), _ptr(v2), uh.data_ptr(), _u_layout(uh), _ptr(bias), b1.data_ptr(), _ptr(b2), umax, ws.data_ptr(), need,
+                                             _ptr(sync), G, C.byref(t), None if gcall is None else C.byref(gcall), C.byref(d), stream())
+    L.check(rc, "mf_conv2d_wino_gn_apply_f16x2_l")
     out._mf_split, out._mf_bound = outs, ob
     if want_wino:
         out._mf_wino, out._mf_wino_bound = ov, ovb
diff --git a/medfusion_amd/lib.py b/medfusion_amd/lib.py
--- a/medfusion_amd/lib.py
+++ b/medfusion_amd/lib.py
@@ -118,6 +118,12 @@
     "mf_wino_group_ok": (_I, [C.POINTER(MfConvDesc), C.POINTER(MfConvDesc)]),
     "mf_conv2d_wino_gn_apply_f16x2": (_I, [c_fp, c_fp, c_fp, c_fp, c_fp, c_fp, _F, c_fp, _SZ, c_fp, _I, C.POINTER(MfWinoTail), C.POINTER(MfConvF16x2Call),
                                            C.POINTER(MfConvDesc), c_fp]),
+    "mf_wino_upanel_default": (_I, []),
+    "mf_wino_tile_weight_bytes": (_SZ, [_I, _I]),
+    "mf_wino_tile_weight_f16x2": (_I, [c_fp, c_fp, _I, _I, c_fp]),
+    "mf_conv2d_wino_f16x2_l": (_I, [c_fp, c_fp, c_fp, _I, c_fp, c_fp, c_fp, c_fp, _F, c_fp, _SZ, c_fp, c_fp, _I, C.POINTER(MfConvDesc), c_fp]),
+    "mf_conv2d_wino_gn_apply_f16x2_l": (_I, [c_fp, c_fp, c_fp, _I, c_fp, c_fp, c_fp, _F, c_fp, _SZ, c_fp, _I, C.POINTER(MfWinoTail), C.POINTER(MfConvF16x2Call),
+                                             C.POINTER(MfConvDesc), c_fp]),
     "mf_maxabs_rows_slots": (_I, [_I64]),
     "mf_maxabs_rows_f32": (_I, [c_fp, c_fp, c_fp, _I, _I64, c_fp]),
     "mf_bound_finalize_f32": (_I, [c_fp, c_fp, _I, _I, c_fp]),
```

Result: no change. 41.72, median of 6 (+0.7%).
